# linjieli222/HERO

Hardware: AMD Instinct MI355X
Metric: videos/sec training step, HERO-base TVR-shaped batch (higher is better)
Workload: dtype bf16; 1 GPU; configs[1]: HERO-base TVR finetune micro-step (train-tvr-8gpu.json shapes: 32 videos x 60 frames, 15 subs x (4 frames + 20 tokens), 15-token query; vfeat 4352; fwd + VSM loss + bwd, all-reduce/clip/AdamW every 2nd micro-step); global_batch=32, parallelism=dp1, grad_accum=2, launch=hipGraph replay, input=one batch resident in HBM

## Files before the change

hero_amd/_lib.py:

```python
import ctypes as C
import os

import torch

_HERE = os.path.dirname(os.path.abspath(__file__))
LIB_PATH = os.environ.get("HERO_HIP_LIB") or os.path.join(_HERE, "libhero_hip.so")

ABI_VERSION = 3
F32, BF16 = 0, 1
LAYOUT_K, LAYOUT_O = 0, 1
ACT_NONE, ACT_GELU, ACT_RELU, ACT_GELU_BWD, ACT_RELU_BWD, ACT_GELU_DG, ACT_MUL_AUX = 0, 1, 2, 3, 4, 5, 6

EXPORTS = [
    "hero_last_error", "hero_abi_version", "hero_abi_struct_count", "hero_abi_struct_bytes", "hero_gemm", "hero_gemm_splits", "hero_fold_slabs", "hero_wgrad_group", "hero_wgrad_batch_plan", "hero_wgrad_batch", "hero_prof_enable", "hero_prof_read", "hero_probe_mfma", "hero_probe_hbm", "hero_gemm_force_config", "hero_layernorm_fwd",
    "hero_layernorm_bwd_workspace_bytes", "hero_layernorm_bwd", "hero_colsum_workspace_bytes",
    "hero_colsum", "hero_colsum_multi", "hero_colsum_multi_workspace_bytes", "hero_layernorm_bwd_blocks", "hero_attention_fwd", "hero_attention_bwd", "hero_attention_max_len", "hero_attention_max_packed_len", "hero_attention_stats_ok", "hero_attention_force_ppw",
    "hero_gather_rows", "hero_inverse_first", "hero_csr_gather_sum", "hero_scatter_add_rows", "hero_segment_sort_workspace_bytes", "hero_scatter_add_sorted_workspace_bytes", "hero_segment_sort", "hero_scatter_add_sorted", "hero_cast", "hero_transpose_cast", "hero_copy_multi",
    "hero_relu_bwd", "hero_gelu_bwd", "hero_add", "hero_sumsq", "hero_adamw", "hero_adamw_multi", "hero_adamw_multi_chunk",
    "hero_query_pool_fwd", "hero_query_pool_bwd", "hero_rownorm_fwd", "hero_rownorm_bwd", "hero_score_max_fwd",
    "hero_score_max_bwd", "hero_rank_loss", "hero_sums_scaled", "hero_st_ed_fwd", "hero_st_ed_bwd", "hero_st_ed_bwd_workspace_bytes",
    "hero_cross_entropy_fwd", "hero_cross_entropy_bwd", "hero_qa_pool_fwd", "hero_qa_pool_bwd",
    "hero_topk_rows", "hero_st_ed_probs", "hero_moment_topk", "hero_moment_nms", "hero_first_hit",
    "hero_collate_subs", "hero_collate_clip_mask", "hero_collate_frame_map", "hero_collate_gather_feats", "hero_derive_multi",
    "hero_comm_available", "hero_comm_unique_id", "hero_comm_init", "hero_comm_destroy", "hero_comm_rank", "hero_comm_world",
    "hero_comm_allreduce_buckets", "hero_comm_broadcast", "hero_comm_allgather", "hero_comm_allgather_var",
]


class Dropout(C.Structure):
    _fields_ = [("seed_ptr", C.c_void_p), ("site", C.c_uint64),
                ("threshold16", C.c_uint32), ("scale", C.c_float)]


class GemmEpilogue(C.Structure):
    _fields_ = [("bias", C.c_void_p), ("residual", C.c_void_p), ("aux", C.c_void_p),
                ("act", C.c_int), ("out_f32", C.c_int), ("beta", C.c_float),
                ("split_k", C.c_int), ("dropout", Dropout), ("colsum", C.c_void_p), ("colsum_partial", C.c_int), ("pad_", C.c_int), ("split_stride", C.c_longlong)]


class CrossEntropy(C.Structure):
    _fields_ = [("logits", C.c_void_p), ("labels", C.c_void_p), ("loss", C.c_void_p), ("lse", C.c_void_p),
                ("dloss", C.c_void_p), ("dlogits", C.c_void_p), ("rows", C.c_int), ("cols", C.c_int),
                ("ld", C.c_int), ("dtype", C.c_int), ("inv_temp", C.c_float), ("ignore_index", C.c_int64)]


class Derive(C.Structure):
    _fields_ = [("src", C.c_void_p), ("dst", C.c_void_p), ("n", C.c_int64), ("mode", C.c_int), ("p0", C.c_int),
                ("p1", C.c_int), ("p2", C.c_int)]


DERIVE_MASK_ADD, DERIVE_F32, DERIVE_I32, DERIVE_FLAT_GATHER = 0, 1, 2, 3


class WgradProblem(C.Structure):
    _fields_ = [("dy", C.c_void_p), ("x", C.c_void_p), ("dw", C.c_void_p), ("M", C.c_int), ("N", C.c_int),
                ("ld_dy", C.c_int), ("ld_x", C.c_int), ("ld_dw", C.c_int), ("split_hint", C.c_int), ("dbias", C.c_void_p)]


class LnFwd(C.Structure):
    _fields_ = [("x", C.c_void_p), ("tab", C.c_void_p * 3), ("idx", C.c_void_p * 3),
                ("gamma", C.c_void_p), ("beta", C.c_void_p), ("y", C.c_void_p),
                ("pre", C.c_void_p), ("mean", C.c_void_p), ("rstd", C.c_void_p),
                ("rows", C.c_int), ("cols", C.c_int), ("eps", C.c_float),
                ("x_dtype", C.c_int), ("y_dtype", C.c_int), ("dropout", Dropout)]


class LnBwd(C.Structure):
    _fields_ = [("x", C.c_void_p), ("dy", C.c_void_p), ("gamma", C.c_void_p),
                ("mean", C.c_void_p), ("rstd", C.c_void_p), ("dx", C.c_void_p),
                ("dx_dropped", C.c_void_p), ("dgamma", C.c_void_p), ("dbeta", C.c_void_p),
                ("grad_beta", C.c_float), ("workspace", C.c_void_p),
                ("rows", C.c_int), ("cols", C.c_int), ("x_dtype", C.c_int), ("dtype", C.c_int),
                ("dropout_out", Dropout), ("dropout_in", Dropout), ("dbias_in", C.c_void_p), ("defer_fold", C.c_int)]


class Colsum(C.Structure):
    _fields_ = [("src", C.c_void_p), ("dst", C.c_void_p), ("rows", C.c_int), ("cols", C.c_int), ("ld", C.c_int),
                ("dtype", C.c_int), ("beta", C.c_float), ("row_cols", C.c_int), ("dst_rows", C.c_void_p)]


class Attn(C.Structure):
    _fields_ = [("qkv", C.c_void_p), ("mask", C.c_void_p), ("ctx", C.c_void_p),
                ("probs", C.c_void_p), ("dctx", C.c_void_p), ("dqkv", C.c_void_p),
                ("S", C.c_int), ("L", C.c_int), ("H", C.c_int), ("scale", C.c_float),
                ("dtype", C.c_int), ("dropout", Dropout), ("seq_off", C.c_void_p), ("stats", C.c_void_p)]


class AdamW(C.Structure):
    _fields_ = [("p", C.c_void_p), ("g", C.c_void_p), ("m", C.c_void_p), ("v", C.c_void_p),
                ("n", C.c_size_t), ("lr", C.c_float), ("beta1", C.c_float), ("beta2", C.c_float),
                ("eps", C.c_float), ("weight_decay", C.c_float), ("step", C.c_int),
                ("grad_sumsq", C.c_void_p), ("max_grad_norm", C.c_float),
                ("grad_scale", C.c_float), ("shadow", C.c_void_p)]


class TensorDesc(C.Structure):
    _fields_ = [("p", C.c_void_p), ("g", C.c_void_p), ("m", C.c_void_p), ("v", C.c_void_p),
                ("n", C.c_uint64), ("group", C.c_int32), ("step_lag", C.c_int32)]


class AdamWGroup(C.Structure):
    _fields_ = [("lr", C.c_float), ("beta1", C.c_float), ("beta2", C.c_float), ("eps", C.c_float),
                ("weight_decay", C.c_float)]


class AdamWMulti(C.Structure):
    _fields_ = [("descs", C.c_void_p), ("chunk_tensor", C.c_void_p), ("chunk_index", C.c_void_p),
                ("n_chunks", C.c_int), ("groups", AdamWGroup * 8), ("step", C.c_int),
                ("grad_sumsq", C.c_void_p), ("max_grad_norm", C.c_float), ("grad_scale", C.c_float),
                ("step_ptr", C.c_void_p), ("lr_ptr", C.c_void_p), ("tensor_steps", C.c_void_p), ("n_tensors", C.c_int)]


class CopyDesc(C.Structure):
    _fields_ = [("src", C.c_void_p), ("dst", C.c_void_p), ("rows", C.c_int32), ("cols", C.c_int32),
                ("ldd", C.c_int32), ("transpose", C.c_int32), ("dst_dtype", C.c_int32), ("pad_", C.c_int32)]


class QueryPool(C.Structure):
    _fields_ = [("q", C.c_void_p), ("mask", C.c_void_p), ("w", C.c_void_p), ("pooled", C.c_void_p),
                ("att", C.c_void_p), ("dpooled", C.c_void_p), ("dq", C.c_void_p), ("dw", C.c_void_p),
                ("B", C.c_int), ("L", C.c_int), ("D", C.c_int), ("dtype", C.c_int)]


class RowNorm(C.Structure):
    _fields_ = [("x", C.c_void_p), ("y", C.c_void_p), ("rnorm", C.c_void_p), ("dy", C.c_void_p),
                ("dx", C.c_void_p), ("rows", C.c_int), ("cols", C.c_int), ("x_dtype", C.c_int),
                ("eps", C.c_float)]


class ScoreMax(C.Structure):
    _fields_ = [("s", C.c_void_p), ("mask", C.c_void_p), ("out", C.c_void_p), ("arg", C.c_void_p),
                ("ds_ctx", C.c_void_p), ("ds_q", C.c_void_p), ("gc", C.c_void_p), ("gq", C.c_void_p),
                ("qn", C.c_void_p), ("cn", C.c_void_p), ("dqn", C.c_void_p), ("dcn", C.c_void_p),
                ("M", C.c_int), ("N", C.c_int), ("L", C.c_int), ("D", C.c_int), ("n0", C.c_int),
                ("n_own", C.c_int), ("ld_s", C.c_int), ("gc_scale", C.c_float), ("gq_scale", C.c_float)]


class RankLoss(C.Structure):
    _fields_ = [("s", C.c_void_p), ("loss_ctx_rows", C.c_void_p), ("loss_q_rows", C.c_void_p),
                ("ds_ctx", C.c_void_p), ("ds_q", C.c_void_p), ("nq", C.c_int), ("nv", C.c_int),
                ("margin", C.c_float), ("lse", C.c_int), ("hard", C.c_int), ("pool", C.c_int),
                ("hard_w", C.c_float), ("easy_w", C.c_float)]


class StEd(C.Structure):
    _fields_ = [("q2", C.c_void_p), ("ctx", C.c_void_p), ("mask", C.c_void_p), ("w_st", C.c_void_p),
                ("w_ed", C.c_void_p), ("targets", C.c_void_p), ("loss_rows", C.c_void_p),
                ("p_st", C.c_void_p), ("p_ed", C.c_void_p), ("sim", C.c_void_p), ("g", C.c_void_p),
                ("dq2", C.c_void_p), ("dctx", C.c_void_p), ("dw_st", C.c_void_p), ("dw_ed", C.c_void_p),
                ("B", C.c_int), ("L", C.c_int), ("D", C.c_int), ("K", C.c_int), ("dtype", C.c_int), ("g_scale", C.c_float),
                ("ws", C.c_void_p)]


class CommBucket(C.Structure):
    _fields_ = [("buf", C.c_void_p), ("count", C.c_size_t), ("dtype", C.c_int), ("pad_", C.c_int)]


ABI_STRUCTS = [Dropout, GemmEpilogue, WgradProblem, LnFwd, LnBwd, Colsum, Attn, AdamW, TensorDesc, AdamWGroup, AdamWMulti,
               CopyDesc, QueryPool, RowNorm, ScoreMax, RankLoss, StEd, CrossEntropy, Derive, CommBucket]


def abi_struct_sizes():
    return {st.__name__: C.sizeof(st) for st in ABI_STRUCTS}


_lib = None


def lib():
    global _lib
    if _lib is None:
        if not os.path.exists(LIB_PATH):
            raise RuntimeError(
                "hero_amd: %s is missing. Build it with `python -m hero_amd.build` "
                "(needs hipcc; cross-compiles for gfx950 without a GPU). There is no fallback "
                "path." % LIB_PATH)
        L = C.CDLL(LIB_PATH)
        L.hero_last_error.restype = C.c_char_p
        have = L.hero_abi_version()
        if have != ABI_VERSION:
            raise RuntimeError("hero_amd: %s reports ABI version %d, this binding was written against %d (struct layouts "
                               "differ: rebuild with `python -m hero_amd.build --force`)" % (LIB_PATH, have, ABI_VERSION))
        L.hero_abi_struct_bytes.argtypes = [C.c_int]
        if L.hero_abi_struct_count() != len(ABI_STRUCTS):
            raise RuntimeError("hero_amd: %s declares %d ABI structs, this binding mirrors %d" % (LIB_PATH, L.hero_abi_struct_count(), len(ABI_STRUCTS)))
        bad = [(st.__name__, C.sizeof(st), L.hero_abi_struct_bytes(i)) for i, st in enumerate(ABI_STRUCTS)
               if C.sizeof(st) != L.hero_abi_struct_bytes(i)]
        if bad:
            raise RuntimeError("hero_amd: struct layouts differ from %s (name, binding bytes, library bytes): %s" % (LIB_PATH, bad))
        L.hero_layernorm_bwd_workspace_bytes.restype = C.c_size_t
        L.hero_colsum_workspace_bytes.restype = C.c_size_t
        L.hero_colsum_multi_workspace_bytes.restype = C.c_size_t
        L.hero_colsum_multi_workspace_bytes.argtypes = [C.POINTER(Colsum), C.c_int]
        L.hero_colsum_multi.argtypes = [C.POINTER(Colsum), C.c_int, C.c_void_p, C.c_void_p]
        L.hero_layernorm_bwd_blocks.argtypes = [C.c_int]
        L.hero_gemm.argtypes = [C.c_void_p, C.c_void_p, C.c_void_p] + [C.c_int] * 9 + [
            C.POINTER(GemmEpilogue), C.c_void_p]
        L.hero_gemm_splits.argtypes = [C.c_int, C.c_int, C.c_int]
        L.hero_fold_slabs.argtypes = [C.c_void_p, C.c_int, C.c_size_t, C.c_void_p, C.c_size_t, C.c_int, C.c_void_p]
        L.hero_wgrad_group.argtypes = [C.POINTER(WgradProblem), C.c_int, C.c_int, C.c_int, C.c_void_p]
        L.hero_wgrad_batch_plan.argtypes = [C.POINTER(WgradProblem), C.c_int, C.c_int, C.c_void_p, C.c_int]
        L.hero_wgrad_batch.argtypes = [C.POINTER(WgradProblem), C.c_int, C.c_int, C.c_int, C.c_void_p, C.c_int, C.c_void_p]
        L.hero_prof_enable.argtypes = [C.c_int]
        L.hero_prof_read.argtypes = [C.c_int, C.POINTER(C.c_double), C.POINTER(C.c_double),
                                     C.POINTER(C.c_longlong)]
        L.hero_probe_mfma.argtypes = [C.c_void_p, C.c_size_t, C.POINTER(C.c_double), C.POINTER(C.c_double), C.c_void_p]
        L.hero_probe_hbm.argtypes = [C.c_void_p, C.c_void_p, C.c_size_t, C.POINTER(C.c_double), C.POINTER(C.c_double), C.c_void_p]
        L.hero_layernorm_fwd.argtypes = [C.POINTER(LnFwd), C.c_void_p]
        L.hero_layernorm_bwd.argtypes = [C.POINTER(LnBwd), C.c_void_p]
        L.hero_layernorm_bwd_workspace_bytes.argtypes = [C.c_int, C.c_int]
        L.hero_colsum_workspace_bytes.argtypes = [C.c_int, C.c_int]
        L.hero_colsum.argtypes = [C.c_void_p, C.c_void_p, C.c_int, C.c_int, C.c_int, C.c_int,
                                  C.c_float, C.c_void_p, C.c_void_p]
        L.hero_attention_fwd.argtypes = [C.POINTER(Attn), C.c_void_p]
        L.hero_attention_bwd.argtypes = [C.POINTER(Attn), C.c_void_p]
        L.hero_attention_stats_ok.argtypes = [C.c_int, C.c_int]
        L.hero_attention_force_ppw.argtypes = [C.c_int]
        L.hero_attention_max_len.argtypes = [C.c_int, C.c_int]
        L.hero_attention_max_packed_len.argtypes = [C.c_int]
        L.hero_gather_rows.argtypes = [C.c_void_p, C.c_void_p, C.c_void_p, C.c_void_p,
                                       C.c_int, C.c_int, C.c_int, C.c_void_p]
        L.hero_inverse_first.argtypes = [C.c_void_p, C.c_int, C.c_void_p, C.c_int, C.c_int, C.c_void_p]
        L.hero_csr_gather_sum.argtypes = [C.c_void_p, C.c_void_p, C.c_void_p, C.c_void_p,
                                          C.c_int, C.c_int, C.c_int, C.c_void_p]
        L.hero_scatter_add_rows.argtypes = [C.c_void_p, C.c_void_p, C.c_void_p, C.c_void_p,
                                            C.c_int, C.c_int, C.c_int, C.c_int, C.c_int, C.c_void_p]
        L.hero_segment_sort_workspace_bytes.argtypes = [C.c_int]
        L.hero_segment_sort_workspace_bytes.restype = C.c_size_t
        L.hero_segment_sort.argtypes = [C.c_void_p, C.c_int, C.c_int, C.c_int, C.c_void_p, C.c_void_p, C.c_void_p]
        L.hero_scatter_add_sorted_workspace_bytes.argtypes = [C.c_int, C.c_int]
        L.hero_scatter_add_sorted_workspace_bytes.restype = C.c_size_t
        L.hero_scatter_add_sorted.argtypes = [C.c_void_p, C.c_void_p, C.c_void_p, C.c_void_p, C.c_int, C.c_int, C.c_int, C.c_int,
                                              C.c_void_p, C.c_void_p]
        L.hero_st_ed_bwd_workspace_bytes.argtypes = [C.c_int]
        L.hero_st_ed_bwd_workspace_bytes.restype = C.c_size_t
        L.hero_cast.argtypes = [C.c_void_p, C.c_void_p, C.c_size_t, C.c_int, C.c_int, C.c_void_p]
        L.hero_transpose_cast.argtypes = [C.c_void_p, C.c_void_p, C.c_int, C.c_int, C.c_int, C.c_int,
                                          C.c_void_p]
        L.hero_relu_bwd.argtypes = [C.c_void_p, C.c_void_p, C.c_void_p, C.c_size_t, C.c_int,
                                    C.c_void_p]
        L.hero_gelu_bwd.argtypes = L.hero_relu_bwd.argtypes
        L.hero_add.argtypes = [C.c_void_p, C.c_void_p, C.c_void_p, C.c_size_t, C.c_int, C.c_void_p]
        L.hero_sumsq.argtypes = [C.c_void_p, C.c_size_t, C.c_void_p, C.c_void_p, C.c_void_p]
        L.hero_adamw.argtypes = [C.POINTER(AdamW), C.c_void_p]
        L.hero_adamw_multi.argtypes = [C.POINTER(AdamWMulti), C.c_void_p]
        L.hero_copy_multi.argtypes = [C.c_void_p, C.c_void_p, C.c_void_p, C.c_int, C.c_void_p]
        for fn, st in (("hero_query_pool_fwd", QueryPool), ("hero_query_pool_bwd", QueryPool),
                       ("hero_rownorm_fwd", RowNorm), ("hero_rownorm_bwd", RowNorm),
                       ("hero_score_max_fwd", ScoreMax), ("hero_score_max_bwd", ScoreMax),
                       ("hero_rank_loss", RankLoss), ("hero_st_ed_fwd", StEd), ("hero_st_ed_bwd", StEd)):
            getattr(L, fn).argtypes = [C.POINTER(st), C.c_void_p]
        L.hero_sums_scaled.argtypes = [C.c_void_p, C.c_int, C.c_int, C.POINTER(C.c_float), C.c_void_p, C.c_void_p]
        L.hero_topk_rows.argtypes = [C.c_void_p, C.c_int, C.c_int, C.c_int, C.c_int, C.c_float, C.c_void_p, C.c_void_p, C.c_void_p]
        L.hero_st_ed_probs.argtypes = [C.c_void_p, C.c_longlong] + [C.c_void_p] * 4 + [C.c_int] * 5 + [C.c_void_p] * 3
        L.hero_moment_topk.argtypes = [C.c_void_p] * 3 + [C.c_int] * 6 + [C.c_void_p] * 3
        L.hero_moment_nms.argtypes = [C.c_void_p] * 3 + [C.c_int, C.c_int, C.c_double, C.c_int, C.c_int] + [C.c_void_p] * 3
        L.hero_first_hit.argtypes = [C.c_void_p] * 3 + [C.c_int] * 3 + [C.c_void_p, C.c_void_p, C.c_float, C.c_void_p, C.c_int, C.c_void_p, C.c_void_p]
        L.hero_collate_subs.argtypes = [C.c_void_p] * 4 + [C.c_int] * 3 + [C.c_void_p]
        L.hero_collate_gather_feats.argtypes = [C.c_void_p] * 7 + [C.c_int] * 5 + [C.c_void_p]
        L.hero_derive_multi.argtypes = [C.POINTER(Derive), C.c_int, C.c_void_p]
        L.hero_collate_clip_mask.argtypes = [C.c_void_p, C.c_void_p, C.c_int, C.c_int, C.c_void_p]
        L.hero_collate_frame_map.argtypes = [C.c_void_p] * 7 + [C.c_int] * 4 + [C.c_void_p]
        L.hero_cross_entropy_fwd.argtypes = [C.POINTER(CrossEntropy), C.c_void_p]
        L.hero_cross_entropy_bwd.argtypes = [C.POINTER(CrossEntropy), C.c_void_p]
        L.hero_qa_pool_fwd.argtypes = [C.c_void_p] * 8 + [C.c_int] * 6 + [C.c_void_p]
        L.hero_qa_pool_bwd.argtypes = [C.c_void_p] * 11 + [C.c_int] * 6 + [C.c_void_p]
        L.hero_comm_unique_id.argtypes = [C.c_void_p]
        L.hero_comm_init.argtypes = [C.c_void_p, C.c_int, C.c_int, C.POINTER(C.c_void_p)]
        L.hero_comm_destroy.argtypes = [C.c_void_p]
        L.hero_comm_rank.argtypes = [C.c_void_p]
        L.hero_comm_world.argtypes = [C.c_void_p]
        L.hero_comm_allreduce_buckets.argtypes = [C.c_void_p, C.POINTER(CommBucket), C.c_int, C.c_void_p]
        L.hero_comm_broadcast.argtypes = [C.c_void_p, C.c_void_p, C.c_size_t, C.c_int, C.c_void_p]
        L.hero_comm_allgather.argtypes = [C.c_void_p, C.c_void_p, C.c_void_p, C.c_size_t, C.c_void_p]
        L.hero_comm_allgather_var.argtypes = [C.c_void_p, C.c_void_p, C.c_void_p, C.POINTER(C.c_size_t), C.c_void_p]
        _lib = L
    return _lib


def check(rc):
    if rc != 0:
        raise RuntimeError("libhero_hip: %s (code %d)" % (lib().hero_last_error().decode(), rc))


def dt(t):
    if t.dtype == torch.float32:
        return F32
    if t.dtype == torch.bfloat16:
        return BF16
    raise TypeError("hero_amd: unsupported dtype %s (float32 / bfloat16 only)" % t.dtype)


def ptr(t):
    if t is None:
        return None
    if not t.is_cuda:
        raise RuntimeError("hero_amd: tensor is on %s; the HIP path needs CUDA/ROCm tensors and has "
                           "no CPU fallback" % t.device)
    if not t.is_contiguous():
        raise RuntimeError("hero_amd: non-contiguous tensor passed to a HIP kernel")
    return t.data_ptr()


_raw_stream = getattr(torch._C, "_cuda_getCurrentRawStream", None)
_cur_device = getattr(torch._C, "_cuda_getDevice", None)


def stream():
    if _raw_stream is not None and _cur_device is not None:
        return _raw_stream(_cur_device())
    return torch.cuda.current_stream().cuda_stream


def no_dropout():
    return Dropout(None, 0, 0, 1.0)
```

hero_amd/build.py:

```python
import os
import shutil
import subprocess
import sys
from concurrent.futures import ThreadPoolExecutor

HERE = os.path.dirname(os.path.abspath(__file__))
CSRC = os.path.join(HERE, "csrc")
OBJ = os.path.join(CSRC, "_obj")
LIB = os.path.join(HERE, "libhero_hip.so")
SOURCES = ["api.cpp", "comm.cpp", "gemm.hip", "gemm_ws.hip", "layernorm.hip", "attention.hip", "attention_mfma.hip", "attention_mfma_long.hip", "rows.hip", "head.hip", "qa_pool.hip", "retrieval.hip", "postproc.hip", "loss.hip", "collate.hip", "probe.hip"]
FLAGS = ["--offload-arch=gfx950", "-O3", "-std=c++17", "-fPIC", "-Wall", "-Wno-unused-function",
         "-ffp-contract=off"]


def _hipcc():
    exe = shutil.which("hipcc") or "/opt/rocm/bin/hipcc"
    if not os.path.exists(exe):
        raise RuntimeError("hipcc not found: cannot build libhero_hip.so")
    return exe


def _stale(target, deps):
    if not os.path.exists(target):
        return True
    t = os.path.getmtime(target)
    return any(os.path.getmtime(d) > t for d in deps)


def build(force=False, verbose=False):
    os.makedirs(OBJ, exist_ok=True)
    hipcc = _hipcc()
    headers = [os.path.join(CSRC, "common.h"), os.path.join(CSRC, "gemm_args.h"), os.path.join(CSRC, "gemm_ws_common.h"), os.path.join(CSRC, "attn_mfma.h"),
               os.path.join(os.path.dirname(HERE), "include", "hero_hip.h")]
    jobs = []
    objs = []
    for src in SOURCES:
        s = os.path.join(CSRC, src)
        o = os.path.join(OBJ, os.path.splitext(src)[0] + ".o")
        objs.append(o)
        if force or _stale(o, [s] + headers):
            jobs.append([hipcc, "-x", "hip"] + FLAGS + ["-c", s, "-o", o])

    def run(cmd):
        if verbose:
            print(" ".join(cmd), flush=True)
        r = subprocess.run(cmd, capture_output=True, text=True)
        if r.returncode != 0:
            raise RuntimeError("hipcc failed:\n%s\n%s" % (" ".join(cmd), r.stderr[-4000:]))
        if verbose and r.stderr.strip():
            print(r.stderr, file=sys.stderr)

    for f in os.listdir(OBJ):
        if f.endswith(".o") and os.path.join(OBJ, f) not in objs:
            os.remove(os.path.join(OBJ, f))
    with ThreadPoolExecutor(max_workers=4) as ex:
        list(ex.map(run, jobs))
    if jobs or force or _stale(LIB, objs):
        run([hipcc, "--offload-arch=gfx950", "-shared", "-fPIC", "-o", LIB] + objs + ["-ldl"])
    return LIB


if __name__ == "__main__":
    print(build(force="--force" in sys.argv, verbose=True))
```

hero_amd/csrc/gemm.hip:

```cpp
#include "gemm_args.h"
#include <vector>

namespace hero {

typedef __attribute__((ext_vector_type(8))) short bf16x8_t;
typedef __attribute__((ext_vector_type(16))) float f32x16_t;

__device__ __forceinline__ int swz(int row) { return (row ^ (row >> 3)) & 7; }

template <typename T> struct Tr;
template <> struct Tr<bf16_t> { static constexpr int BK = 64, EPC = 8; };
template <> struct Tr<float>  { static constexpr int BK = 32, EPC = 4; };

template <int WM_, int WN_, int TM_, int TN_> struct Cfg {
  static constexpr int WM = WM_, WN = WN_, TM = TM_, TN = TN_;
  static constexpr int NT = 64 * WM * WN;
  static constexpr int BM = WM * TM * 32, BN = WN * TN * 32;
  static constexpr int A_BYTES = BM * 128, B_BYTES = BN * 128, STAGE = A_BYTES + B_BYTES;
  static constexpr int EPI_ROWS = BM < 128 ? BM : (BM % 128 == 0 ? 128 : BM / 2);
  static constexpr int EPI_BYTES = EPI_ROWS * BN * 4;
  static constexpr int LDS = 2 * STAGE > EPI_BYTES ? 2 * STAGE : EPI_BYTES;
};

template <typename T, int LAY, int R, int NT> struct Stage;
// ... 757 lines not shown
  return check_launch("hero_gemm");
}

static int pick_cfg(int M, int N, int split, bool k_contig) {
  if (g_force_cfg >= 0 && g_force_cfg < 8) return g_force_cfg;
  if (!k_contig || split != 1) return 0;
  const long long t128 = (long long)((M + 127) / 128) * ((N + 127) / 128);
  if (t128 <= 192) return 3;
  if (t128 > 512 && t128 <= 700 && (long long)((M + 191) / 192) * ((N + 127) / 128) <= 512) return 1;
  const long long tiles = (long long)((M + 255) / 256) * ((N + 255) / 256);
  const long long rounds = (tiles + 255) / 256;
  return (tiles >= 256 && tiles * 10 >= rounds * 256 * 9) ? 2 : 0;
}

static int g_use_glds = 1;

#define HERO_GLDS_INST(T, CF)                                                       \
  template __global__ void gemm_glds_kernel<T, CF, EK_GENERIC>(GemmArgs);           \
  template __global__ void gemm_glds_kernel<T, CF, 0>(GemmArgs);                    \
  template __global__ void gemm_glds_kernel<T, CF, EK_BIAS>(GemmArgs);              \
  template __global__ void gemm_glds_kernel<T, CF, EK_BIAS | EK_RES | EK_DROP>(GemmArgs); \
  template __global__ void gemm_glds_kernel<T, CF, EK_BIAS | EK_GELU>(GemmArgs);    \
  template __global__ void gemm_glds_kernel<T, CF, EK_RES>(GemmArgs);               \
  template __global__ void gemm_glds_kernel<T, CF, EK_GELU_BWD>(GemmArgs);
HERO_GLDS_INST(bf16_t, Cfg128)
HERO_GLDS_INST(bf16_t, Cfg256)
HERO_GLDS_INST(bf16_t, Cfg64)
HERO_GLDS_INST(bf16_t, Cfg192)
template __global__ void gemm_glds_kernel<float, Cfg192, EK_GENERIC>(GemmArgs);
template __global__ void gemm_glds_kernel<float, Cfg64, EK_GENERIC>(GemmArgs);
template __global__ void gemm_glds_kernel<float, Cfg128, EK_GENERIC>(GemmArgs);
template __global__ void gemm_glds_kernel<float, Cfg256, EK_GENERIC>(GemmArgs);

template <typename T, typename CF, int EK>
static int launch_glds_ek(GemmArgs g, hipStream_t s) {
  HERO_ENSURE_LDS((&gemm_glds_kernel<T, CF, EK>), GldsRing<CF>::LDS, "gemm_glds_kernel");
  g.tiles_m = (g.M + CF::BM - 1) / CF::BM;
  g.tiles_n = (g.N + CF::BN - 1) / CF::BN;
  const int split = g.epi.split_k > 1 ? g.epi.split_k : 1;
  const int grid = g.tiles_m * g.tiles_n * split;
  ProfSlot* ps = nullptr;
  hipEvent_t e0 = nullptr, e1 = nullptr;
  if (g_prof_on) {
    ps = &g_prof[(sizeof(T) == 2 ? 4 : 0)];
    if (ps->flops.size() < 16384 && hipEventCreate(&e0) == hipSuccess && hipEventCreate(&e1) == hipSuccess) {
      (void)hipEventRecord(e0, s);
    } else {
      ps = nullptr;
    }
  }
  hipLaunchKernelGGL((gemm_glds_kernel<T, CF, EK>), dim3(grid), dim3(CF::NT), GldsRing<CF>::LDS, s, g);
  if (ps) {
    (void)hipEventRecord(e1, s);
    ps->ev.push_back(e0);
    ps->ev.push_back(e1);
    ps->flops.push_back(2.0 * (double)g.M * (double)g.N * (double)g.K);
  }
  return check_launch("hero_gemm(glds)");
}

template <typename T, typename CF>
static int launch_glds(const GemmArgs& g, hipStream_t s) {
  const HeroGemmEpilogue& e = g.epi;
  if constexpr (sizeof(T) == 2) if (!e.out_f32 && e.split_k <= 1) {
    const bool b = e.bias != nullptr, r = e.residual != nullptr, d = e.dropout.threshold16 != 0;
    if (e.act == HERO_ACT_NONE && b && !r && !d) return launch_glds_ek<T, CF, EK_BIAS>(g, s);
    if (e.act == HERO_ACT_NONE && b && r) return launch_glds_ek<T, CF, EK_BIAS | EK_RES | EK_DROP>(g, s);
    if ((e.act == HERO_ACT_GELU || e.act == HERO_ACT_GELU_DG) && b && !r && !d) return launch_glds_ek<T, CF, EK_BIAS | EK_GELU>(g, s);
    if (e.act == HERO_ACT_NONE && !b && !r && !d) return launch_glds_ek<T, CF, 0>(g, s);
    if (e.act == HERO_ACT_NONE && !b && r && !d) return launch_glds_ek<T, CF, EK_RES>(g, s);
    if ((e.act == HERO_ACT_GELU_BWD || e.act == HERO_ACT_MUL_AUX) && !b && !r && !d) return launch_glds_ek<T, CF, EK_GELU_BWD>(g, s);
  }
  return launch_glds_ek<T, CF, EK_GENERIC>(g, s);
}

static int launch_glds_tr(GemmArgs g, hipStream_t s) {
  typedef Cfg<2, 2, 2, 2> CF;
  g.tiles_m = (g.M + CF::BM - 1) / CF::BM;
  g.tiles_n = (g.N + CF::BN - 1) / CF::BN;
  const int split = g.epi.split_k > 1 ? g.epi.split_k : 1;
  const int grid = g.tiles_m * g.tiles_n * split;
  ProfSlot* ps = nullptr;
  hipEvent_t e0 = nullptr, e1 = nullptr;
  if (g_prof_on) {
    ps = &g_prof[7];
    if (ps->flops.size() < 16384 && hipEventCreate(&e0) == hipSuccess && hipEventCreate(&e1) == hipSuccess) {
      (void)hipEventRecord(e0, s);
    } else {
      ps = nullptr;
    }
  }
  HERO_ENSURE_LDS(&gemm_glds_tr_kernel, 65536, "gemm_glds_tr_kernel");
  hipLaunchKernelGGL(gemm_glds_tr_kernel, dim3(grid), dim3(256), 65536, s, g);
  if (ps) {
    (void)hipEventRecord(e1, s);
    ps->ev.push_back(e0);
    ps->ev.push_back(e1);
    ps->flops.push_back(2.0 * (double)g.M * (double)g.N * (double)g.K);
  }
  return check_launch("hero_gemm(glds_tr)");
}

template <typename T, int AL, int BL>
static int launch_cfg(const GemmArgs& g, int cfg, hipStream_t s) {
  if (AL == HERO_LAYOUT_O && BL == HERO_LAYOUT_O && sizeof(T) == 2 && g_use_glds && g.K > 0 && g.k_per_split % 64 == 0)
    return launch_glds_tr(g, s);
  if (AL == HERO_LAYOUT_K && BL == HERO_LAYOUT_K && g_use_glds && g.K > 0 && g.K % Tr<T>::BK == 0 &&
      g.k_per_split % Tr<T>::BK == 0) {
    if (cfg == 2) return launch_glds<T, Cfg256>(g, s);
    if (cfg == 3) return launch_glds<T, Cfg64>(g, s);
    if (cfg == 1) return launch_glds<T, Cfg192>(g, s);
    return launch_glds<T, Cfg128>(g, s);
  }
  if (cfg == 2) return launch<T, AL, BL, Cfg256>(g, s);
  return launch<T, AL, BL, Cfg128>(g, s);
}

template <typename T>
static int dispatch(const GemmArgs& g, int al, int bl, int cfg, hipStream_t s) {
  if (al == HERO_LAYOUT_K && bl == HERO_LAYOUT_K) return launch_cfg<T, HERO_LAYOUT_K, HERO_LAYOUT_K>(g, cfg, s);
  if (al == HERO_LAYOUT_K && bl == HERO_LAYOUT_O) return launch_cfg<T, HERO_LAYOUT_K, HERO_LAYOUT_O>(g, cfg, s);
  if (al == HERO_LAYOUT_O && bl == HERO_LAYOUT_O) return launch_cfg<T, HERO_LAYOUT_O, HERO_LAYOUT_O>(g, cfg, s);
  if (al == HERO_LAYOUT_O && bl == HERO_LAYOUT_K) return launch_cfg<T, HERO_LAYOUT_O, HERO_LAYOUT_K>(g, cfg, s);
  set_error("hero_gemm: bad layout (%d, %d)", al, bl);
  return HERO_ERR_ARG;
}

}

using namespace hero;

template <int CTRL, int ROW_MASK>
__device__ __forceinline__ float dpp_add(float v) {
  return v + __builtin_bit_cast(float, __builtin_amdgcn_update_dpp(0, __builtin_bit_cast(int, v), CTRL, ROW_MASK, 0xf, false));
}
__device__ __forceinline__ float wave_sum_lane63(float v) {
  v = dpp_add<0xb1, 0xf>(v);
  v = dpp_add<0x4e, 0xf>(v);
  v = dpp_add<0x124, 0xf>(v);
  v = dpp_add<0x128, 0xf>(v);
  v = dpp_add<0x142, 0xa>(v);
  v = dpp_add<0x143, 0xc>(v);
  return v;
}

__global__ __launch_bounds__(256) void gemm_skinny_f32_kernel(const float* __restrict__ A, const float* __restrict__ B, float* __restrict__ C,
                                                              const float* __restrict__ bias, int M, int N, int K, int lda, int ldb, int ldc) {
  extern __shared__ __attribute__((aligned(16))) char smem_skinny[];
  float* xs = reinterpret_cast<float*>(smem_skinny);
  constexpr int KC = 1024;
  const int lane = threadIdx.x & 63, wave = threadIdx.x >> 6;
  const int n0 = (blockIdx.x * 4 + wave) * 2;
  const bool live = n0 < N, two = n0 + 1 < N;
  float acc0[32], acc1[32];
#pragma unroll
  for (int m = 0; m < 32; ++m) acc0[m] = acc1[m] = 0.f;
  const float* b0 = B + (size_t)(live ? n0 : 0) * ldb;
  const float* b1 = B + (size_t)(two ? n0 + 1 : (live ? n0 : 0)) * ldb;
  for (int kc = 0; kc < K; kc += KC) {
    const int kw = min(KC, K - kc);
    float4 w0[4], w1[4];
#pragma unroll
    for (int j = 0; j < 4; ++j) {
      const int k = min(lane * 4 + j * 256, kw - 4);
      w0[j] = *reinterpret_cast<const float4*>(b0 + kc + k);
      w1[j] = *reinterpret_cast<const float4*>(b1 + kc + k);
    }
    if (kc) __syncthreads();
    {
      const int k = threadIdx.x * 4;
      const bool in = k < kw;
      const float* src = A + kc + (in ? k : 0);
      float* dst = in ? xs + k : xs + 32 * kw;
      const int dstride = in ? kw : 0;
#pragma unroll
      for (int m0 = 0; m0 < 32; m0 += 16) {
        float4 t[16];
#pragma unroll
        for (int j = 0; j < 16; ++j) t[j] = *reinterpret_cast<const float4*>(src + (size_t)(m0 + j < M ? m0 + j : M - 1) * lda);
#pragma unroll
        for (int j = 0; j < 16; ++j) *reinterpret_cast<float4*>(dst + (m0 + j) * dstride) = t[j];
      }
    }
    __syncthreads();
    if (live) {
#pragma unroll
      for (int j = 0; j < 4; ++j) {
        const int k = lane * 4 + j * 256;
        if (k < kw) {
#pragma unroll
          for (int m0 = 0; m0 < 32; m0 += 16) {
            float4 xv[16];
#pragma unroll
            for (int q = 0; q < 16; ++q) xv[q] = *reinterpret_cast<const float4*>(xs + (m0 + q) * kw + k);
            __builtin_amdgcn_sched_barrier(0);
#pragma unroll
            for (int q = 0; q < 16; ++q) {
              const float4 x = xv[q];
              acc0[m0 + q] = fmaf(x.w, w0[j].w, fmaf(x.z, w0[j].z, fmaf(x.y, w0[j].y, fmaf(x.x, w0[j].x, acc0[m0 + q]))));
              acc1[m0 + q] = fmaf(x.w, w1[j].w, fmaf(x.z, w1[j].z, fmaf(x.y, w1[j].y, fmaf(x.x, w1[j].x, acc1[m0 + q]))));
            }
            __builtin_amdgcn_sched_barrier(0);
          }
        }
      }
    }
  }
  if (!live) return;
  float v0 = 0.f, v1 = 0.f;
#pragma unroll
  for (int m = 0; m < 32; ++m) {
    const float s0 = __builtin_bit_cast(float, __builtin_amdgcn_readlane(__builtin_bit_cast(int, wave_sum_lane63(acc0[m])), 63));
    const float s1 = __builtin_bit_cast(float, __builtin_amdgcn_readlane(__builtin_bit_cast(int, wave_sum_lane63(acc1[m])), 63));
    v0 = lane == m ? s0 : v0;
    v1 = lane == m ? s1 : v1;
  }
  if (lane < M) {
    C[(size_t)lane * ldc + n0] = v0 + (bias ? bias[n0] : 0.f);
    if (two) C[(size_t)lane * ldc + n0 + 1] = v1 + (bias ? bias[n0 + 1] : 0.f);
  }
}

extern "C" int hero_gemm(const void* A, const void* B, void* C, int M, int N, int K, int lda, int ldb, int ldc,
                         int a_layout, int b_layout, int dtype, const HeroGemmEpilogue* epi, hero_stream_t stream) {
  HERO_REQUIRE(A && B && C && epi, "hero_gemm: null pointer");
  HERO_REQUIRE(dtype == HERO_F32 || dtype == HERO_BF16, "hero_gemm: bad dtype %d", dtype);
  if (M <= 0 || N <= 0) return HERO_OK;
  HERO_REQUIRE(K >= 0, "hero_gemm: K < 0");
  const int vec = dtype == HERO_BF16 ? 8 : 4;
  HERO_REQUIRE(N % 4 == 0 && ldc % 4 == 0, "hero_gemm: N (%d) and ldc (%d) must be multiples of 4", N, ldc);
  HERO_REQUIRE(lda % vec == 0 && ldb % vec == 0, "hero_gemm: lda/ldb (%d, %d) must be multiples of %d", lda, ldb, vec);
  HERO_REQUIRE(a_layout == HERO_LAYOUT_K ? K % vec == 0 : M % vec == 0,
               "hero_gemm: A contiguous dim must be a multiple of %d (M=%d K=%d layout=%d)", vec, M, K, a_layout);
  HERO_REQUIRE(b_layout == HERO_LAYOUT_K ? K % vec == 0 : N % vec == 0,
               "hero_gemm: B contiguous dim must be a multiple of %d (N=%d K=%d layout=%d)", vec, N, K, b_layout);
  HERO_REQUIRE((((uintptr_t)A | (uintptr_t)B | (uintptr_t)C) & 15) == 0, "hero_gemm: operands must be 16-byte aligned");
  HERO_REQUIRE(!epi->residual || (((uintptr_t)epi->residual) & 7) == 0, "hero_gemm: residual misaligned");
  HERO_REQUIRE(!(epi->act == HERO_ACT_GELU || epi->act == HERO_ACT_GELU_BWD || epi->act == HERO_ACT_RELU_BWD || epi->act == HERO_ACT_GELU_DG ||
                 epi->act == HERO_ACT_MUL_AUX) || epi->aux,
               "hero_gemm: activation %d needs aux", epi->act);
  HERO_REQUIRE(!epi->colsum || (epi->split_k <= 1 && !epi->out_f32), "hero_gemm: epilogue.colsum excludes split_k / out_f32");
  HERO_REQUIRE(epi->split_stride == 0 || (epi->split_k > 1 && epi->split_stride >= (long long)(M - 1) * ldc + N),
               "hero_gemm: split_stride needs split_k > 1 and slabs that hold [M, ldc]");
  GemmArgs g;
  g.A = A; g.B = B; g.C = C;
  g.M = M; g.N = N; g.K = K; g.lda = lda; g.ldb = ldb; g.ldc = ldc;
  g.tiles_m = g.tiles_n = 0;
  g.group = g_group ? g_group : (N >= 2560 ? 16 : (N <= 1024 ? 4 : 8));
  g.epi = *epi;
  const int bk = dtype == HERO_BF16 ? 64 : 32;
  const bool k_contig = a_layout == HERO_LAYOUT_K && b_layout == HERO_LAYOUT_K;
  hipStream_t s = static_cast<hipStream_t>(stream);
  if (dtype == HERO_F32 && k_contig && M <= 32 && K >= 256 && g_force_cfg == -1 && epi->act == HERO_ACT_NONE && !epi->residual && !epi->colsum &&
      !epi->out_f32 && epi->split_k <= 1 && epi->dropout.threshold16 == 0) {
    void* tok = gemm_prof_begin(3, s);
    const int lds = 32 * (K < 1024 ? K : 1024) * 4 + 16;
    HERO_ENSURE_LDS(&gemm_skinny_f32_kernel, 32 * 1024 * 4 + 16, "gemm_skinny_f32_kernel");
    hipLaunchKernelGGL(gemm_skinny_f32_kernel, dim3((N + 7) / 8), dim3(256), lds, s, static_cast<const float*>(A), static_cast<const float*>(B),
                       static_cast<float*>(C), epi->bias, M, N, K, lda, ldb, ldc);
    gemm_prof_end(tok, 2.0 * (double)M * (double)N * (double)K, s);
    return check_launch("hero_gemm(skinny f32)");
  }
  if (dtype == HERO_BF16) {
    const int rc = gemm_ws_run(A, B, C, M, N, K, lda, ldb, ldc, a_layout, b_layout, *epi, g_force_cfg, s);
    if (rc != -1) return rc;
  }
  if (epi->split_k > 1) {
    HERO_REQUIRE(epi->out_f32 && epi->act == HERO_ACT_NONE && !epi->bias && !epi->residual && epi->dropout.threshold16 == 0,
                 "hero_gemm: split_k supports only a plain fp32 accumulate epilogue");
    const int ktiles = (K + bk - 1) / bk;
    int split = epi->split_k < ktiles ? epi->split_k : ktiles;
    if (split > 1) {
      const int per = (ktiles + split - 1) / split;
      split = (ktiles + per - 1) / per;
      if (split > 1) {
        if (epi->split_stride == 0 && epi->beta != 1.f) {
          hipLaunchKernelGGL(scale_f32_kernel, dim3(1024), dim3(256), 0, s, static_cast<float*>(C), M, N, ldc, epi->beta);
          const int rc = check_launch("hero_gemm(scale)");
          if (rc) return rc;
        }
        g.k_per_split = per * bk;
        g.epi.split_k = split;
        const int cfg = pick_cfg(M, N, split, k_contig);
        return dtype == HERO_BF16 ? dispatch<bf16_t>(g, a_layout, b_layout, cfg, s) : dispatch<float>(g, a_layout, b_layout, cfg, s);
      }
    }
  }
  g.k_per_split = K > 0 ? ((K + bk - 1) / bk) * bk : bk;
  g.epi.split_k = 1;
  const int cfg = pick_cfg(M, N, 1, k_contig);
  return dtype == HERO_BF16 ? dispatch<bf16_t>(g, a_layout, b_layout, cfg, s) : dispatch<float>(g, a_layout, b_layout, cfg, s);
}

extern "C" int hero_gemm_splits(int K, int split_k, int dtype) {
  const int bk = dtype == HERO_BF16 ? 64 : 32;
  const int ktiles = (K + bk - 1) / bk;
  int split = split_k < ktiles ? split_k : ktiles;
  if (split <= 1) return 1;
  const int per = (ktiles + split - 1) / split;
  return (ktiles + per - 1) / per;
}

extern "C" int hero_gemm_force_config(int cfg) {
  if (cfg >= 8 && cfg <= 14 && cfg != 11 && cfg != 12) {
    g_force_cfg = cfg;
    g_use_glds = 1;
    g_group = 0;
    return HERO_OK;
  }
  g_force_cfg = cfg >= 0 ? (cfg & 3) : -1;
  g_use_glds = cfg >= 0 ? !(cfg & 4) : 1;
  g_group = cfg >= 0 ? (cfg >> 8) : 0;
  return HERO_OK;
}

extern "C" int hero_prof_enable(int on) {
  for (auto& p : g_prof) {
    for (hipEvent_t e : p.ev) (void)hipEventDestroy(e);
    p.ev.clear();
    p.flops.clear();
  }
  g_prof_on = on != 0;
  return HERO_OK;
}
extern "C" int hero_prof_read(int slot, double* total_ms, double* total_flops, long long* launches) {
  HERO_REQUIRE(slot >= 0 && slot < 11 && total_ms && total_flops && launches, "hero_prof_read: bad arguments");
  ProfSlot& p = g_prof[slot];
  double ms = 0.0, fl = 0.0;
  for (size_t i = 0; i < p.flops.size(); ++i) {
    float t = 0.f;
    if (hipEventSynchronize(p.ev[2 * i + 1]) != hipSuccess || hipEventElapsedTime(&t, p.ev[2 * i], p.ev[2 * i + 1]) != hipSuccess) {
      set_error("hero_prof_read: event query failed");
      return HERO_ERR_LAUNCH;
    }
    ms += t;
    fl += p.flops[i];
  }
  *total_ms = ms;
  *total_flops = fl;
  *launches = (long long)p.flops.size();
  return HERO_OK;
}
```

hero_amd/csrc/gemm_ws.hip:

```cpp
#include <stdlib.h>
#include <type_traits>

#include "gemm_ws_common.h"

namespace hero {
namespace ws {

template <int TM, int TN, bool TR, int EK>
__global__ __launch_bounds__(512) __attribute__((amdgpu_waves_per_eu(2, 2))) void gemm_ws_kernel(WsArgs g) {
  typedef Geo<TM, TN> G;
  extern __shared__ __attribute__((aligned(16))) char smem[];
  const int lane = threadIdx.x & 63;
  const int wave = __builtin_amdgcn_readfirstlane(threadIdx.x >> 6);
  const int nwg = gridDim.x;
  int wg;
  {
    const int bid = blockIdx.x, q = nwg >> 3, r = nwg & 7, xcd = bid & 7, loc = bid >> 3;
    wg = (xcd < r ? xcd * (q + 1) : r * (q + 1) + (xcd - r) * q) + loc;
  }

  if (wave >= 4) {
    Loader<G, TR> ld(g, smem, wg, nwg, wave - 4, lane);
    constexpr int AHEAD = (G::NSG - 2) * G::PW;
    bool more = ld.issue();
#pragma unroll
    for (int k = 0; k < G::NSG - 2; ++k) more = ld.issue();
    if (more) wait_vm<AHEAD>(); else wait_vm<0>();
    __builtin_amdgcn_s_barrier();
    unsigned slot = 0;
    int item_no = 0;
    for (int cit = wg; cit < g.nwork; cit += nwg, ++item_no) {
      const Item ic = item_coord<G>(g, cit);
      WS_T(item_no, 0, wave, lane);
      for (int t = 0; t < ic.nk; ++t) {
        if (ld.issue()) wait_vm<AHEAD>(); else wait_vm<0>();
        __builtin_amdgcn_s_barrier();
        if (t + 1 < ic.nk) { slot += G::STAGE; if (slot == G::NSG * G::STAGE) slot = 0; }
      }
      WS_T(item_no, 1, wave, lane);
#ifndef HERO_WS_NOEPI
      if constexpr (!TR) epilogue_rows<G, EK, false>(g, ic, smem, slot, nullptr, wave, lane, item_no);
#endif
      slot += G::STAGE; if (slot == G::NSG * G::STAGE) slot = 0;
    }
    return;
  }

  const int wm = wave >> 1, wn = wave & 1;
  const int arow0 = wm * TM * 32, brow0 = wn * TN * 32;
  unsigned ao[TM], bo[TN];
  if (!TR) {
    const int r = lane & 31, kg = lane >> 5;
#pragma unroll
    for (int i = 0; i < TM; ++i) { const int ra = arow0 + i * 32 + r; ao[i] = ra * 128 + ((kg ^ swz_k(ra)) << 4); }
#pragma unroll
    for (int j = 0; j < TN; ++j) { const int rb = brow0 + j * 32 + r; bo[j] = G::A_BYTES + rb * 128 + ((kg ^ swz_k(rb)) << 4); }
  } else {
    const int p = lane & 15, gq = (lane >> 4) & 1, kg = lane >> 5;
    const int krow = kg * 8 + (p >> 2);
#pragma unroll
    for (int i = 0; i < TM; ++i) {
      const int col = arow0 + i * 32 + gq * 16 + 4 * (p & 3);
      ao[i] = krow * (G::BM * 2) + ((((col >> 3) ^ swz_o<G::BM * 2>(krow)) << 4) | ((col & 7) * 2));
    }
#pragma unroll
    for (int j = 0; j < TN; ++j) {
      const int col = brow0 + j * 32 + gq * 16 + 4 * (p & 3);
      bo[j] = G::A_BYTES + krow * (G::BN * 2) + ((((col >> 3) ^ swz_o<G::BN * 2>(krow)) << 4) | ((col & 7) * 2));
    }
  }
  bf16x8_t a0[TM], b0[TN], a1[TM], b1[TN];
  auto ldf = [&](bf16x8_t (&a)[TM], bf16x8_t (&b)[TN], const char* st, int ks) {
    typedef __attribute__((address_space(3))) bf16x4_t* lp_t;
    auto ra = [&](int i) {
      if (!TR) {
        a[i] = *reinterpret_cast<const bf16x8_t*>(st + (ao[i] ^ (ks << 5)));
      } else {
        const char* q = st + ao[i] + ks * 16 * (G::BM * 2);
        const bf16x4_t lo = __builtin_amdgcn_ds_read_tr16_b64_v4i16((lp_t)(q));
        const bf16x4_t hi = __builtin_amdgcn_ds_read_tr16_b64_v4i16((lp_t)(q + 4 * (G::BM * 2)));
        a[i] = bf16x8_t{lo[0], lo[1], lo[2], lo[3], hi[0], hi[1], hi[2], hi[3]};
      }
    };
    auto rb = [&](int j) {
      if (!TR) {
        b[j] = *reinterpret_cast<const bf16x8_t*>(st + (bo[j] ^ (ks << 5)));
      } else {
        const char* q = st + bo[j] + ks * 16 * (G::BN * 2);
        const bf16x4_t lo = __builtin_amdgcn_ds_read_tr16_b64_v4i16((lp_t)(q));
        const bf16x4_t hi = __builtin_amdgcn_ds_read_tr16_b64_v4i16((lp_t)(q + 4 * (G::BN * 2)));
        b[j] = bf16x8_t{lo[0], lo[1], lo[2], lo[3], hi[0], hi[1], hi[2], hi[3]};
      }
    };
    if (!TR) {
      ra(0);
#pragma unroll
      for (int j = 0; j < TN; ++j) rb(j);
#pragma unroll
      for (int i = 1; i < TM; ++i) ra(i);
    } else {
      ra(0);
#pragma unroll
      for (int j = 0; j < TN; ++j) rb(j);
#pragma unroll
      for (int i = 1; i < TM; ++i) ra(i);
    }
  };
  f32x16_t acc[TM][TN];
  auto mma = [&](const bf16x8_t (&a)[TM], const bf16x8_t (&b)[TN]) {
#pragma unroll
    for (int i = 0; i < TM; ++i)
#pragma unroll
      for (int j = 0; j < TN; ++j) {
        if (!TR) acc[i][j] = __builtin_amdgcn_mfma_f32_32x32x16_bf16(b[j], a[i], acc[i][j], 0, 0, 0);
        else acc[i][j] = __builtin_amdgcn_mfma_f32_32x32x16_bf16(a[i], b[j], acc[i][j], 0, 0, 0);
      }
  };

  __builtin_amdgcn_s_setprio(2);
  __builtin_amdgcn_s_barrier();
  unsigned curo = 0;
  if (wg < g.nwork) ldf(a0, b0, smem, 0);
  int item_no = 0;
  for (int cit = wg; cit < g.nwork; cit += nwg, ++item_no) {
    const Item ic = item_coord<G>(g, cit);
    WS_T(item_no, 0, wave, lane);
#pragma unroll
    for (int i = 0; i < TM; ++i)
#pragma unroll
      for (int j = 0; j < TN; ++j)
#pragma unroll
        for (int e = 0; e < 16; ++e) acc[i][j][e] = 0.f;
    const bool more_items = cit + nwg < g.nwork;
    unsigned last = curo;
    for (int t = 0; t < ic.nk; ++t) {
      const char* cur = smem + curo;
      last = curo;
      curo += G::STAGE;
      if (curo == G::NSG * G::STAGE) curo = 0;
      const char* nxt = smem + curo;
      constexpr int NRD = TR ? 2 * (TM + TN) : TM + TN;
      ldf(a1, b1, cur, 1);
      mma(a0, b0);
      WS_INTERLEAVE(TM * TN, NRD);
      __builtin_amdgcn_sched_barrier(0);
      ldf(a0, b0, cur, 2);
      mma(a1, b1);
      WS_INTERLEAVE(TM * TN, NRD);
      __builtin_amdgcn_sched_barrier(0);
      ldf(a1, b1, cur, 3);
      mma(a0, b0);
      WS_INTERLEAVE(TM * TN, NRD);
      __builtin_amdgcn_sched_barrier(0);
      wait_lds();
      __builtin_amdgcn_s_barrier();
      __builtin_amdgcn_sched_barrier(0);
      ldf(a0, b0, nxt, 0);
      mma(a1, b1);
      WS_INTERLEAVE(TM * TN, NRD);
      __builtin_amdgcn_sched_barrier(0);
    }
    if constexpr (!TR) {
      __builtin_amdgcn_s_setprio(0);
      WS_T(item_no, 1, wave, lane);
#ifndef HERO_WS_NOEPI
      epilogue_rows<G, EK, true>(g, ic, smem, last, acc, wave, lane, item_no);
#else
      {
        float sum = 0.f;
#pragma unroll
        for (int i = 0; i < TM; ++i)
#pragma unroll
          for (int j = 0; j < TN; ++j)
#pragma unroll
            for (int e = 0; e < 16; ++e) sum += acc[i][j][e];
        if (sum == 1.2345e-30f) static_cast<bf16_t*>(g.C)[lane] = (bf16_t)1;
      }
#endif
      __builtin_amdgcn_s_setprio(2);
      if (more_items) ldf(a0, b0, smem + curo, 0);
    } else {
      float* C = static_cast<float*>(g.C);
#pragma unroll
      for (int i = 0; i < TM; ++i)
#pragma unroll
        for (int j = 0; j < TN; ++j) {
          const int gn = ic.n0 + brow0 + j * 32 + (lane & 31);
#pragma unroll
          for (int r = 0; r < 16; ++r) {
            const int gm = ic.m0 + arow0 + i * 32 + (r & 3) + 8 * (r >> 2) + 4 * (lane >> 5);
            if (gm < g.M && gn < g.N) atomicAdd(C + (size_t)gm * g.ldc + gn, acc[i][j][r]);
          }
        }
    }
  }
}

struct WsgProb {
  const bf16_t* A;
  const bf16_t* B;
  float* C;
  int M, N, lda, ldb, ldc, tiles_n, tile0;
};
struct WsgArgs {
  WsgProb p[4];
  int nprob, K, ksteps, total_tiles;
};
struct Seg { int prob, m0, n0, k0, nk; };

template <typename G>
__device__ __forceinline__ Seg seg_at(const WsgArgs& g, int pos, int end) {
  const int tile = pos / g.ksteps, k0 = pos - tile * g.ksteps;
  int pi = 0;
#pragma unroll
  for (int q = 1; q < 4; ++q)
    if (q < g.nprob && tile >= g.p[q].tile0) pi = q;
  const int t = tile - g.p[pi].tile0;
  Seg s;
  s.prob = pi;
  s.m0 = (t / g.p[pi].tiles_n) * G::BM;
  s.n0 = (t % g.p[pi].tiles_n) * G::BN;
  s.k0 = k0;
  s.nk = min(g.ksteps - k0, end - pos);
  return s;
}

__global__ __launch_bounds__(512) __attribute__((amdgpu_waves_per_eu(2, 2))) void gemm_wsg_kernel(WsgArgs g) {
  typedef Geo<3, 3> G;
  constexpr int TM = 3, TN = 3;
  extern __shared__ __attribute__((aligned(16))) char smem[];
  const int lane = threadIdx.x & 63;
  const int wave = __builtin_amdgcn_readfirstlane(threadIdx.x >> 6);
  const int nwg = gridDim.x;
  int wg;
  {
    const int bid = blockIdx.x, q = nwg >> 3, r = nwg & 7, xcd = bid & 7, loc = bid >> 3;
    wg = (xcd < r ? xcd * (q + 1) : r * (q + 1) + (xcd - r) * q) + loc;
  }
  const long long total = (long long)g.total_tiles * g.ksteps;
  const int start = (int)(total * wg / nwg), end = (int)(total * (wg + 1) / nwg);
  if (start >= end) return;

  if (wave >= 4) {
    const int w = wave - 4;
    constexpr int CA = G::BM / 8, CB = G::BN / 8;
    int pos = start;
    Seg sg = seg_at<G>(g, pos, end);
    int ik = 0;
    unsigned goa[G::PA], gob[G::PB];
    const char* pa = nullptr;
    const char* pb = nullptr;
    unsigned ra_left = 0, rb_left = 0, sa = 0, sb = 0, fill = 0;
    auto setup = [&]() {
      const WsgProb& P = g.p[sg.prob];
#pragma unroll
      for (int i = 0; i < G::PA; ++i) {
        const int id = (w * G::PA + i) * 64 + lane, row = id / CA, c = (id % CA) ^ swz_o<G::BM * 2>(row);
        goa[i] = (unsigned)row * (unsigned)P.lda * 2u + (c << 4);
      }
#pragma unroll
      for (int i = 0; i < G::PB; ++i) {
        const int id = (w * G::PB + i) * 64 + lane, row = id / CB, c = (id % CB) ^ swz_o<G::BN * 2>(row);
        gob[i] = (unsigned)row * (unsigned)P.ldb * 2u + (c << 4);
      }
      const int kb = sg.k0 * 64;
      pa = reinterpret_cast<const char*>(P.A + (size_t)kb * P.lda + sg.m0);
      pb = reinterpret_cast<const char*>(P.B + (size_t)kb * P.ldb + sg.n0);
      ra_left = (unsigned)(((size_t)(g.K - kb) * P.lda - sg.m0) * 2);
      rb_left = (unsigned)(((size_t)(g.K - kb) * P.ldb - sg.n0) * 2);
      sa = 64u * (unsigned)P.lda * 2u;
      sb = 64u * (unsigned)P.ldb * 2u;
    };
    setup();
    auto issue = [&]() -> bool {
      if (pos >= end) return false;
      char* buf = smem + fill;
      const __amdgpu_buffer_rsrc_t ra = __builtin_amdgcn_make_buffer_rsrc(const_cast<char*>(pa), 0, ra_left, 0x00020000);
      const __amdgpu_buffer_rsrc_t rb = __builtin_amdgcn_make_buffer_rsrc(const_cast<char*>(pb), 0, rb_left, 0x00020000);
#pragma unroll
      for (int i = 0; i < G::PA; ++i)
        __builtin_amdgcn_raw_ptr_buffer_load_lds(ra, HERO_LDS_PTR(buf + (w * G::PA + i) * 1024), 16, goa[i], 0, 0, HERO_WS_LOAD_AUX_A);
#pragma unroll
      for (int i = 0; i < G::PB; ++i)
        __builtin_amdgcn_raw_ptr_buffer_load_lds(rb, HERO_LDS_PTR(buf + G::A_BYTES + (w * G::PB + i) * 1024), 16, gob[i], 0, 0, HERO_WS_LOAD_AUX_B);
      fill += G::STAGE;
      if (fill == NS * G::STAGE) fill = 0;
      ++pos;
      if (++ik == sg.nk) {
        ik = 0;
        if (pos < end) { sg = seg_at<G>(g, pos, end); setup(); }
      } else {
        pa += sa; pb += sb;
        ra_left = ra_left > sa ? ra_left - sa : 0u;
        rb_left = rb_left > sb ? rb_left - sb : 0u;
      }
      return true;
    };
    issue();
    const bool second = issue();
    if (second) wait_vm<G::PW>(); else wait_vm<0>();
    __builtin_amdgcn_s_barrier();
    for (int u = start; u < end; ++u) {
      if (issue()) wait_vm<G::PW>(); else wait_vm<0>();
      __builtin_amdgcn_s_barrier();
    }
    return;
  }

  const int wm = wave >> 1, wn = wave & 1;
  const int arow0 = wm * TM * 32, brow0 = wn * TN * 32;
  unsigned ao[TM], bo[TN];
  {
    const int p = lane & 15, gq = (lane >> 4) & 1, kg = lane >> 5;
    const int krow = kg * 8 + (p >> 2);
#pragma unroll
    for (int i = 0; i < TM; ++i) {
      const int col = arow0 + i * 32 + gq * 16 + 4 * (p & 3);
      ao[i] = krow * (G::BM * 2) + ((((col >> 3) ^ swz_o<G::BM * 2>(krow)) << 4) | ((col & 7) * 2));
    }
#pragma unroll
    for (int j = 0; j < TN; ++j) {
      const int col = brow0 + j * 32 + gq * 16 + 4 * (p & 3);
      bo[j] = G::A_BYTES + krow * (G::BN * 2) + ((((col >> 3) ^ swz_o<G::BN * 2>(krow)) << 4) | ((col & 7) * 2));
    }
  }
  typedef __attribute__((address_space(3))) bf16x4_t* lp_t;
  bf16x8_t a0[TM], b0[TN], a1[TM], b1[TN];
  auto ldf = [&](bf16x8_t (&a)[TM], bf16x8_t (&b)[TN], const char* st, int ks) {
    auto ra = [&](int i) {
      const char* q = st + ao[i] + ks * 16 * (G::BM * 2);
      const bf16x4_t lo = __builtin_amdgcn_ds_read_tr16_b64_v4i16((lp_t)(q));
      const bf16x4_t hi = __builtin_amdgcn_ds_read_tr16_b64_v4i16((lp_t)(q + 4 * (G::BM * 2)));
      a[i] = bf16x8_t{lo[0], lo[1], lo[2], lo[3], hi[0], hi[1], hi[2], hi[3]};
    };
    ra(0);
#pragma unroll
    for (int j = 0; j < TN; ++j) {
      const char* q = st + bo[j] + ks * 16 * (G::BN * 2);
      const bf16x4_t lo = __builtin_amdgcn_ds_read_tr16_b64_v4i16((lp_t)(q));
      const bf16x4_t hi = __builtin_amdgcn_ds_read_tr16_b64_v4i16((lp_t)(q + 4 * (G::BN * 2)));
      b[j] = bf16x8_t{lo[0], lo[1], lo[2], lo[3], hi[0], hi[1], hi[2], hi[3]};
    }
#pragma unroll
    for (int i = 1; i < TM; ++i) ra(i);
  };
  f32x16_t acc[TM][TN];
  auto mma = [&](const bf16x8_t (&a)[TM], const bf16x8_t (&b)[TN]) {
#pragma unroll
    for (int i = 0; i < TM; ++i)
#pragma unroll
      for (int j = 0; j < TN; ++j) acc[i][j] = __builtin_amdgcn_mfma_f32_32x32x16_bf16(a[i], b[j], acc[i][j], 0, 0, 0);
  };
  __builtin_amdgcn_s_setprio(2);
  __builtin_amdgcn_s_barrier();
  unsigned curo = 0;
  ldf(a0, b0, smem, 0);
  [[maybe_unused]] int seg_no = 0;
  for (int pos = start; pos < end; ++seg_no) {
    const Seg sg = seg_at<G>(g, pos, end);
    WS_T(seg_no, 0, wave, lane);
#pragma unroll
    for (int i = 0; i < TM; ++i)
#pragma unroll
      for (int j = 0; j < TN; ++j)
#pragma unroll
        for (int e = 0; e < 16; ++e) acc[i][j][e] = 0.f;
    for (int t = 0; t < sg.nk; ++t) {
      const char* cur = smem + curo;
      curo += G::STAGE;
      if (curo == NS * G::STAGE) curo = 0;
      const char* nxt = smem + curo;
      ldf(a1, b1, cur, 1);
      mma(a0, b0);
      WS_INTERLEAVE(TM * TN, 2 * (TM + TN));
      __builtin_amdgcn_sched_barrier(0);
      ldf(a0, b0, cur, 2);
      mma(a1, b1);
      WS_INTERLEAVE(TM * TN, 2 * (TM + TN));
      __builtin_amdgcn_sched_barrier(0);
      ldf(a1, b1, cur, 3);
      mma(a0, b0);
      WS_INTERLEAVE(TM * TN, 2 * (TM + TN));
      __builtin_amdgcn_sched_barrier(0);
      wait_lds();
      __builtin_amdgcn_s_barrier();
      __builtin_amdgcn_sched_barrier(0);
      ldf(a0, b0, nxt, 0);
      mma(a1, b1);
      WS_INTERLEAVE(TM * TN, 2 * (TM + TN));
      __builtin_amdgcn_sched_barrier(0);
    }
    pos += sg.nk;
    WS_T(seg_no, 1, wave, lane);
#ifdef HERO_WS_TRACE
    if (blockIdx.x == 0 && lane == 0 && seg_no < 4) g_ws_trace[(seg_no * 16 + 3) * 8 + wave] = (unsigned long long)sg.nk;
#endif
    const WsgProb& P = g.p[sg.prob];
#pragma unroll
    for (int i = 0; i < TM; ++i)
#pragma unroll
      for (int j = 0; j < TN; ++j) {
        const int gn = sg.n0 + brow0 + j * 32 + (lane & 31);
#pragma unroll
        for (int r = 0; r < 16; ++r) {
          const int gm = sg.m0 + arow0 + i * 32 + (r & 3) + 8 * (r >> 2) + 4 * (lane >> 5);
          if (gm < P.M && gn < P.N) atomicAdd(P.C + (size_t)gm * P.ldc + gn, acc[i][j][r]);
        }
      }
    WS_T(seg_no, 14, wave, lane);
  }
}

struct WsbProb {
  const bf16_t* A;
  const bf16_t* B;
  float* C;
  float* colsum;
  int M, N, lda, ldb, ldc, pad_;
};
struct WsbItem { int prob, m0, n0, k0, nk, order, nslices, flag; };
struct WsbArgs {
  const WsbItem* items;
  int* flags;
  int rounds, K, nprob, pad_;
  WsbProb p[HERO_WGRAD_BATCH_MAX];
};

template <typename G, bool COMPUTE>
__device__ __forceinline__ void epilogue_acc(const WsbProb& P, const WsbItem& it, int* flags, char* smem, unsigned slot,
                                             f32x16_t (*acc)[G::TN], int wave, int lane, bool want_cs = false) {
  constexpr int TM = G::TM, TN = G::TN, BN = G::BN, RPP = G::RPP, C8 = G::C8, RPI = G::RPI, ITERS = G::ITERS;
  char* st = smem + slot;
  int tid = threadIdx.x;
  asm volatile("" : "+v"(tid));
  lane = tid & 63;
  wave = __builtin_amdgcn_readfirstlane(tid >> 6);
  const int c8 = tid % C8, r0 = tid / C8;
  const int gn = it.n0 + c8 * 8;
  const bool col_ok = r0 < RPI && gn < P.N;
  const int wm = wave >> 1, wn = wave & 1, l31 = lane & 31, half = lane >> 5;
  const bool plain = it.nslices == 1;
  constexpr bool SPLIT = (RPP == 64 && G::PASSES == TM);
  auto tile_row = [](int p, int row) { return SPLIT ? (row >> 5) * (TM * 32) + p * 32 + (row & 31) : p * RPP + row; };
  const __amdgpu_buffer_rsrc_t rc = __builtin_amdgcn_make_buffer_rsrc(P.C, 0, 0x7ffffff0, 0x00020000);
  if (!plain && it.order > 0) {
    if (lane == 0)
      while (__hip_atomic_load(flags + it.flag, __ATOMIC_RELAXED, __HIP_MEMORY_SCOPE_AGENT) != it.order) __builtin_amdgcn_s_sleep(8);
  }
#pragma unroll
  for (int p = 0; p < G::PASSES; ++p) {
    u32x4_t old0[ITERS], old1[ITERS];
    unsigned voff[ITERS];
    if (plain) {
#pragma unroll
      for (int i = 0; i < ITERS; ++i) {
        const int row = r0 + i * RPI;
        const int gm = it.m0 + tile_row(p, row);
        const bool ok = col_ok && row < RPP && gm < P.M;
        voff[i] = ok ? ((unsigned)gm * (unsigned)P.ldc + (unsigned)gn) * 4u : 0xfffffff0u;
#if defined(HERO_WSB_EPI_NOLOAD) || defined(HERO_WSB_EPI_NOMEM)
        old0[i] = u32x4_t{0u, 0u, 0u, 0u};
        old1[i] = u32x4_t{0u, 0u, 0u, 0u};
#else
        old0[i] = __builtin_amdgcn_raw_buffer_load_b128(rc, voff[i], 0, 0);
        old1[i] = __builtin_amdgcn_raw_buffer_load_b128(rc, voff[i], 16, 0);
#endif
      }
    }
    if constexpr (COMPUTE) {
#pragma unroll
      for (int b = 0; b < RPP / 32; ++b) {
        const int blk = SPLIT ? b * TM + p : p * (RPP / 32) + b;
        if (wm == blk / TM) {
          const int i = blk % TM;
#pragma unroll
          for (int j = 0; j < TN; ++j)
#pragma unroll
            for (int q = 0; q < 4; ++q) {
              const int chunk = (wn * TN * 32 + j * 32 + 8 * q + 4 * half) >> 2;
              const f32x4_t v = {acc[i][j][4 * q], acc[i][j][4 * q + 1], acc[i][j][4 * q + 2], acc[i][j][4 * q + 3]};
              *reinterpret_cast<f32x4_t*>(st + (32 * b + l31) * G::ROWB + ((chunk ^ (l31 & 7)) << 4)) = v;
            }
        }
      }
    }
    wait_lds();
    __builtin_amdgcn_s_barrier();
    if constexpr (!COMPUTE) {
      if (p == 0 && want_cs && tid - 256 < G::BM) {
        const int c = tid - 256, gm = it.m0 + c;
        const float* sp = reinterpret_cast<const float*>(smem + SPARE_OFF);
        const float sum = sp[c];
        if (gm < P.M) {
          if (plain) P.colsum[gm] += sum; else atomicAdd(P.colsum + gm, sum);
        }
      }
    }
    if (plain) {
// ... 15 lines not shown
          }
#ifdef HERO_WSB_EPI_NOMEM
        asm volatile("" ::"v"(v0[0]), "v"(v1[0]), "v"(v0[1]), "v"(v1[1]));
        continue;
#endif
#pragma unroll
        for (int i = 0; i < 2; ++i) {
          __builtin_amdgcn_raw_buffer_store_b128(u32x4_t{__float_as_uint(v0[i][0]), __float_as_uint(v0[i][1]), __float_as_uint(v0[i][2]), __float_as_uint(v0[i][3])}, rc, voff[h + i], 0, HERO_WS_STORE_DW);
          __builtin_amdgcn_raw_buffer_store_b128(u32x4_t{__float_as_uint(v1[i][0]), __float_as_uint(v1[i][1]), __float_as_uint(v1[i][2]), __float_as_uint(v1[i][3])}, rc, voff[h + i], 16, HERO_WS_STORE_DW);
        }
      }
    } else {
      const int col = tid % BN, rr = tid / BN;
      const int gc = it.n0 + col;
      if (tid < 2 * BN && gc < P.N) {
        const unsigned sw = (unsigned)(col >> 2);
#pragma unroll 4
        for (int q = 0; q < RPP / 2; ++q) {
          const int row = 2 * q + rr;
          const int gm = it.m0 + tile_row(p, row);
          const float v = *reinterpret_cast<const float*>(st + row * G::ROWB + (((sw ^ (unsigned)(row & 7))) << 4) + (col & 3) * 4);
          if (gm < P.M) atomicAdd(P.C + (size_t)gm * P.ldc + gc, v);
        }
      }
      if (p == G::PASSES - 1) wait_vm<0>();
    }
    wait_lds();
    __builtin_amdgcn_s_barrier();
  }
  if (!plain && tid == 0)
    __hip_atomic_store(flags + it.flag, it.order + 1 < it.nslices ? it.order + 1 : 0, __ATOMIC_RELAXED, __HIP_MEMORY_SCOPE_AGENT);
}

__global__ __launch_bounds__(512) __attribute__((amdgpu_waves_per_eu(2, 2))) void gemm_wsb_kernel(WsbArgs g) {
  typedef Geo<3, 3> G;
  constexpr int TM = 3, TN = 3;
  extern __shared__ __attribute__((aligned(16))) char smem[];
  const int lane = threadIdx.x & 63;
  const int wave = __builtin_amdgcn_readfirstlane(threadIdx.x >> 6);
  const int nwg = gridDim.x;
  int wg;
  {
    const int bid = blockIdx.x, q = nwg >> 3, r = nwg & 7, xcd = bid & 7, loc = bid >> 3;
    wg = (xcd < r ? xcd * (q + 1) : r * (q + 1) + (xcd - r) * q) + loc;
  }
  auto next_round = [&](int r) {
    while (r < g.rounds && g.items[(size_t)r * nwg + wg].nk == 0) ++r;
    return r;
  };

  if (wave >= 4) {
    const int w = wave - 4;
    constexpr int CA = G::BM / 8, CB = G::BN / 8;
    int lr = next_round(0), ik = 0, lnk = 0;
    unsigned goa[G::PA], gob[G::PB];
    const char* pa = nullptr;
    const char* pb = nullptr;
    unsigned long long ra_left = 0, rb_left = 0;
    unsigned sa = 0, sb = 0, fill = 0;
    auto setup = [&]() {
      const WsbItem it = g.items[(size_t)lr * nwg + wg];
      const WsbProb& P = g.p[it.prob];
      lnk = it.nk;
#pragma unroll
      for (int i = 0; i < G::PA; ++i) {
        const int id = (w * G::PA + i) * 64 + lane, row = id / CA, c = (id % CA) ^ swz_o<G::BM * 2>(row);
        goa[i] = (unsigned)row * (unsigned)P.lda * 2u + (c << 4);
      }
#pragma unroll
      for (int i = 0; i < G::PB; ++i) {
        const int id = (w * G::PB + i) * 64 + lane, row = id / CB, c = (id % CB) ^ swz_o<G::BN * 2>(row);
        gob[i] = (unsigned)row * (unsigned)P.ldb * 2u + (c << 4);
      }
      const int kb = it.k0 * 64;
      pa = reinterpret_cast<const char*>(P.A + (size_t)kb * P.lda + it.m0);
      pb = reinterpret_cast<const char*>(P.B + (size_t)kb * P.ldb + it.n0);
      ra_left = ((unsigned long long)(g.K - kb) * P.lda - it.m0) * 2;
      rb_left = ((unsigned long long)(g.K - kb) * P.ldb - it.n0) * 2;
      sa = 64u * (unsigned)P.lda * 2u;
      sb = 64u * (unsigned)P.ldb * 2u;
    };
    if (lr < g.rounds) setup();
    auto issue = [&]() -> bool {
      if (lr >= g.rounds) return false;
      char* buf = smem + fill;
      const __amdgpu_buffer_rsrc_t ra = __builtin_amdgcn_make_buffer_rsrc(const_cast<char*>(pa), 0, (unsigned)(ra_left < 0xfffffff0ull ? ra_left : 0xfffffff0ull), 0x00020000);
      const __amdgpu_buffer_rsrc_t rb = __builtin_amdgcn_make_buffer_rsrc(const_cast<char*>(pb), 0, (unsigned)(rb_left < 0xfffffff0ull ? rb_left : 0xfffffff0ull), 0x00020000);
#ifndef HERO_WSB_NOLOADS
#pragma unroll
      for (int i = 0; i < G::PA; ++i)
        __builtin_amdgcn_raw_ptr_buffer_load_lds(ra, HERO_LDS_PTR(buf + (w * G::PA + i) * 1024), 16, goa[i], 0, 0, HERO_WS_LOAD_AUX_A);
#pragma unroll
      for (int i = 0; i < G::PB; ++i)
        __builtin_amdgcn_raw_ptr_buffer_load_lds(rb, HERO_LDS_PTR(buf + G::A_BYTES + (w * G::PB + i) * 1024), 16, gob[i], 0, 0, HERO_WS_LOAD_AUX_B);
#else
      (void)ra; (void)rb; (void)buf;
#endif
      fill += G::STAGE;
      if (fill == NS * G::STAGE) fill = 0;
      if (++ik == lnk) {
        ik = 0;
        lr = next_round(lr + 1);
        if (lr < g.rounds) setup();
      } else {
        pa += sa; pb += sb;
        ra_left = ra_left > sa ? ra_left - sa : 0ull;
        rb_left = rb_left > sb ? rb_left - sb : 0ull;
      }
      return true;
    };
    issue();
    const bool second = issue();
    if (second) wait_vm<G::PW>(); else wait_vm<0>();
    __builtin_amdgcn_s_barrier();
    unsigned slot = 0;
    for (int r = next_round(0); r < g.rounds; r = next_round(r + 1)) {
      const WsbItem it = g.items[(size_t)r * nwg + wg];
      const bool want_cs = it.n0 == 0 && g.p[it.prob].colsum != nullptr;
      for (int t = 0; t < it.nk; ++t) {
        const bool more = issue();
        if (more) wait_vm<G::PW>(); else wait_vm<0>();
#ifndef HERO_WSB_NOBAR
        __builtin_amdgcn_s_barrier();
#endif
        if (t + 1 < it.nk) { slot += G::STAGE; if (slot == NS * G::STAGE) slot = 0; }
      }
#ifndef HERO_WSB_NOEPI
      epilogue_acc<G, false>(g.p[it.prob], it, g.flags, smem, slot, nullptr, wave, lane, want_cs);
#endif
      slot += G::STAGE; if (slot == NS * G::STAGE) slot = 0;
    }
    return;
  }

  const int wm = wave >> 1, wn = wave & 1;
  const int arow0 = wm * TM * 32, brow0 = wn * TN * 32;
  unsigned ao[TM], bo[TN];
  {
    const int p = lane & 15, gq = (lane >> 4) & 1, kg = lane >> 5;
    const int krow = kg * 8 + (p >> 2);
#pragma unroll
    for (int i = 0; i < TM; ++i) {
      const int col = arow0 + i * 32 + gq * 16 + 4 * (p & 3);
      ao[i] = krow * (G::BM * 2) + ((((col >> 3) ^ swz_o<G::BM * 2>(krow)) << 4) | ((col & 7) * 2));
    }
#pragma unroll
    for (int j = 0; j < TN; ++j) {
      const int col = brow0 + j * 32 + gq * 16 + 4 * (p & 3);
      bo[j] = G::A_BYTES + krow * (G::BN * 2) + ((((col >> 3) ^ swz_o<G::BN * 2>(krow)) << 4) | ((col & 7) * 2));
    }
  }
  typedef __attribute__((address_space(3))) bf16x4_t* lp_t;
  bf16x8_t a0[TM], b0[TN], a1[TM], b1[TN];
  auto ldf = [&](bf16x8_t (&a)[TM], bf16x8_t (&b)[TN], const char* st, int ks) {
#ifdef HERO_WSB_NOLDF
    return;
#endif
    auto ra = [&](int i) {
      const char* q = st + ao[i] + ks * 16 * (G::BM * 2);
      const bf16x4_t lo = __builtin_amdgcn_ds_read_tr16_b64_v4i16((lp_t)(q));
      const bf16x4_t hi = __builtin_amdgcn_ds_read_tr16_b64_v4i16((lp_t)(q + 4 * (G::BM * 2)));
      a[i] = bf16x8_t{lo[0], lo[1], lo[2], lo[3], hi[0], hi[1], hi[2], hi[3]};
    };
    ra(0);
#pragma unroll
    for (int j = 0; j < TN; ++j) {
      const char* q = st + bo[j] + ks * 16 * (G::BN * 2);
      const bf16x4_t lo = __builtin_amdgcn_ds_read_tr16_b64_v4i16((lp_t)(q));
      const bf16x4_t hi = __builtin_amdgcn_ds_read_tr16_b64_v4i16((lp_t)(q + 4 * (G::BN * 2)));
      b[j] = bf16x8_t{lo[0], lo[1], lo[2], lo[3], hi[0], hi[1], hi[2], hi[3]};
    }
#pragma unroll
    for (int i = 1; i < TM; ++i) ra(i);
  };
  f32x16_t acc[TM][TN];
  f32x16_t accb;
  unsigned selw[TM];
#pragma unroll
  for (int i = 0; i < TM; ++i) selw[i] = ((lane & 31) >> 3) == i ? 0x3f803f80u : 0u;
  auto mma = [&](const bf16x8_t (&a)[TM], const bf16x8_t (&b)[TN], auto cs) {
#ifdef HERO_WSB_NOMFMA
    asm volatile("" ::"v"(a[0]), "v"(b[0]), "v"(a[TM - 1]), "v"(b[TN - 1]));
    return;
#endif
#pragma unroll
    for (int i = 0; i < TM; ++i) {
#pragma unroll
      for (int j = 0; j < TN; ++j) acc[i][j] = __builtin_amdgcn_mfma_f32_32x32x16_bf16(b[j], a[i], acc[i][j], 0, 0, 0);
      if constexpr (decltype(cs)::value) {
        const u32x4_t w4 = {selw[i], selw[i], selw[i], selw[i]};
        accb = __builtin_amdgcn_mfma_f32_32x32x16_bf16(__builtin_bit_cast(bf16x8_t, w4), a[i], accb, 0, 0, 0);
      }
    }
  };
  unsigned curo = 0, last = 0;
  auto k_loop = [&](int nk, auto cs) {
    constexpr int NM = TM * TN + (decltype(cs)::value ? TM : 0);
    for (int t = 0; t < nk; ++t) {
      const char* cur = smem + curo;
      last = curo;
      curo += G::STAGE;
      if (curo == NS * G::STAGE) curo = 0;
      const char* nxt = smem + curo;
      ldf(a1, b1, cur, 1);
      mma(a0, b0, cs);
      WS_INTERLEAVE(NM, 2 * (TM + TN));
      __builtin_amdgcn_sched_barrier(0);
      ldf(a0, b0, cur, 2);
      mma(a1, b1, cs);
      WS_INTERLEAVE(NM, 2 * (TM + TN));
      __builtin_amdgcn_sched_barrier(0);
      ldf(a1, b1, cur, 3);
      mma(a0, b0, cs);
      WS_INTERLEAVE(NM, 2 * (TM + TN));
      __builtin_amdgcn_sched_barrier(0);
      wait_lds();
#ifndef HERO_WSB_NOBAR
      __builtin_amdgcn_s_barrier();
#endif
      __builtin_amdgcn_sched_barrier(0);
      ldf(a0, b0, nxt, 0);
      mma(a1, b1, cs);
      WS_INTERLEAVE(NM, 2 * (TM + TN));
      __builtin_amdgcn_sched_barrier(0);
    }
  };
  __builtin_amdgcn_s_setprio(2);
  __builtin_amdgcn_s_barrier();
  int r = next_round(0);
  if (r < g.rounds) ldf(a0, b0, smem, 0);
  while (r < g.rounds) {
    const WsbItem it = g.items[(size_t)r * nwg + wg];
    const int rn = next_round(r + 1);
    const bool cs_on = wn == 0 && it.n0 == 0 && g.p[it.prob].colsum != nullptr;
#pragma unroll
    for (int i = 0; i < TM; ++i)
#pragma unroll
      for (int j = 0; j < TN; ++j)
#pragma unroll
        for (int e = 0; e < 16; ++e) acc[i][j][e] = 0.f;
    last = curo;
    if (cs_on) {
#pragma unroll
      for (int e = 0; e < 16; ++e) accb[e] = 0.f;
      k_loop(it.nk, std::true_type{});
      float* sp = reinterpret_cast<float*>(smem + SPARE_OFF);
      if (lane < 32) {
#pragma unroll
        for (int i = 0; i < TM; ++i) sp[arow0 + 32 * i + lane] = accb[4 * i];
      }
    } else {
      k_loop(it.nk, std::false_type{});
    }
    __builtin_amdgcn_s_setprio(0);
#ifndef HERO_WSB_NOEPI
    epilogue_acc<G, true>(g.p[it.prob], it, g.flags, smem, last, acc, wave, lane);
#else
#pragma unroll
    for (int i = 0; i < TM; ++i)
#pragma unroll
      for (int j = 0; j < TN; ++j) asm volatile("" ::"v"(acc[i][j]));
#endif
    __builtin_amdgcn_s_setprio(2);
    if (rn < g.rounds) ldf(a0, b0, smem + curo, 0);
    r = rn;
  }
}

#define HERO_WS_INST(TM, TN)                                                                  \
  template __global__ void gemm_ws_kernel<TM, TN, false, 0>(WsArgs);                          \
  template __global__ void gemm_ws_kernel<TM, TN, false, EK_BIAS>(WsArgs);                    \
  template __global__ void gemm_ws_kernel<TM, TN, false, EK_BIAS | EK_RES | EK_DROP>(WsArgs); \
  template __global__ void gemm_ws_kernel<TM, TN, false, EK_BIAS | EK_GELU>(WsArgs);          \
  template __global__ void gemm_ws_kernel<TM, TN, false, EK_RES>(WsArgs);                     \
  template __global__ void gemm_ws_kernel<TM, TN, false, EK_GELU_BWD>(WsArgs);                \
  template __global__ void gemm_ws_kernel<TM, TN, true, 0>(WsArgs);
HERO_WS_INST(3, 3)
HERO_WS_INST(2, 3)

__global__ void ws_scale_f32_kernel(float* c, int M, int N, int ldc, float beta) {
  const size_t n4 = (size_t)N >> 2;
  for (size_t i = blockIdx.x * (size_t)blockDim.x + threadIdx.x; i < (size_t)M * n4; i += (size_t)gridDim.x * blockDim.x) {
    const size_t r = i / n4, c4 = (i - r * n4) * 4;
    float4* p = reinterpret_cast<float4*>(c + r * ldc + c4);
    if (beta == 0.f) {
      *p = make_float4(0.f, 0.f, 0.f, 0.f);
    } else {
      float4 v = *p;
      v.x *= beta; v.y *= beta; v.z *= beta; v.w *= beta;
      *p = v;
    }
  }
}

static int num_cus() {
  static int n = [] {
    int dev = 0, v = 256;
    if (hipGetDevice(&dev) == hipSuccess) (void)hipDeviceGetAttribute(&v, hipDeviceAttributeMultiprocessorCount, dev);
    return v > 0 ? v : 256;
  }();
  return n;
}

template <int TM, int TN, bool TR, int EK>
static int launch(WsArgs g, int slot, hipStream_t s) {
  typedef Geo<TM, TN> G;
  HERO_ENSURE_LDS((&gemm_ws_kernel<TM, TN, TR, EK>), G::LDS, "gemm_ws_kernel");
  const int grid = g.nwork < num_cus() ? g.nwork : num_cus();
  void* tok = gemm_prof_begin(slot, s);
  hipLaunchKernelGGL((gemm_ws_kernel<TM, TN, TR, EK>), dim3(grid), dim3(512), G::LDS, s, g);
  gemm_prof_end(tok, 2.0 * (double)g.M * (double)g.N * (double)g.K, s);
  return check_launch("hero_gemm(ws)");
}

template <int TM, int TN>
static int launch_kk(const WsArgs& g, hipStream_t s) {
  const HeroGemmEpilogue& e = g.epi;
  const bool b = e.bias != nullptr, r = e.residual != nullptr, d = e.dropout.threshold16 != 0;
  if (e.colsum != nullptr && e.act != HERO_ACT_GELU_BWD && e.act != HERO_ACT_MUL_AUX) return -1;
  if (e.act == HERO_ACT_NONE && b && !r && !d) return launch<TM, TN, false, EK_BIAS>(g, TM == 3 ? 8 : 10, s);
  if (e.act == HERO_ACT_NONE && b && r) return launch<TM, TN, false, EK_BIAS | EK_RES | EK_DROP>(g, TM == 3 ? 8 : 10, s);
  if ((e.act == HERO_ACT_GELU || e.act == HERO_ACT_GELU_DG) && b && !r && !d) return launch<TM, TN, false, EK_BIAS | EK_GELU>(g, TM == 3 ? 8 : 10, s);
  if (e.act == HERO_ACT_RELU && b && !r && !d && e.aux) return launch<TM, TN, false, EK_BIAS | EK_GELU>(g, TM == 3 ? 8 : 10, s);
  if constexpr (TM == 1) {
    if (e.act == HERO_ACT_RELU && b && r && !d && e.aux) return launch<TM, TN, false, EK_BIAS | EK_GELU | EK_RES>(g, 10, s);
  }
  if (e.act == HERO_ACT_NONE && !b && !r && !d) return launch<TM, TN, false, 0>(g, TM == 3 ? 8 : 10, s);
  if (e.act == HERO_ACT_NONE && !b && r && !d) return launch<TM, TN, false, EK_RES>(g, TM == 3 ? 8 : 10, s);
  if ((e.act == HERO_ACT_GELU_BWD || e.act == HERO_ACT_MUL_AUX) && !b && !r && !d) return launch<TM, TN, false, EK_GELU_BWD>(g, TM == 3 ? 8 : 10, s);
  return -1;
}

}

int gemm_ws_run(const void* A, const void* B, void* C, int M, int N, int K, int lda, int ldb, int ldc, int a_layout,
                int b_layout, const HeroGemmEpilogue& epi, int force_cfg, hipStream_t s) {
  using namespace ws;
  if (force_cfg == 8) return -1;
  if ((force_cfg < 9 || force_cfg > 14 || force_cfg == 11 || force_cfg == 12) && force_cfg != -1) return -1;
  typedef Geo<3, 3> G;
  const bool kk = a_layout == HERO_LAYOUT_K && b_layout == HERO_LAYOUT_K;
  const bool oo = a_layout == HERO_LAYOUT_O && b_layout == HERO_LAYOUT_O;
  if (!kk && !oo) return -1;
  if (K < 64 || N % 8 != 0 || M < 8) return -1;
  if ((force_cfg == 10 || force_cfg == 13 || force_cfg == 14) && !kk) return -1;
  WsArgs g;
  g.A = A; g.B = B; g.C = C;
  g.M = M; g.N = N; g.K = K; g.lda = lda; g.ldb = ldb; g.ldc = ldc;
  g.tiles_m = (M + G::BM - 1) / G::BM;
  g.tiles_n = (N + G::BN - 1) / G::BN;
  g.epi = epi;
  const int ntile = g.tiles_m * g.tiles_n;
  const int cus = num_cus();
  if (kk) {
    if (K % 64 != 0 || epi.out_f32 || epi.split_k > 1) return -1;
    if ((size_t)N * ldb * 2 >= 0x7fffffffull || (size_t)192 * lda * 2 >= 0x7fffffffull || (size_t)192 * ldc * 2 >= 0x7fffffffull) return -1;
    g.nsplit = 1;
    g.k_per_split = K;
    g.group = 8;
    typedef Geo<2, 3> G2;
    const int t23 = ((M + G2::BM - 1) / G2::BM) * g.tiles_n;
    const int r33 = (ntile + cus - 1) / cus, r23 = (t23 + cus - 1) / cus;
    const bool small = force_cfg == 10 || (force_cfg == -1 && r23 * 4 < r33 * 5 && t23 * 5 >= cus * 2);
    if (small) {
      g.tiles_m = (M + G2::BM - 1) / G2::BM;
      g.nwork = t23;
      return launch_kk<2, 3>(g, s);
    }
    if (force_cfg == 13 || force_cfg == 14 || (force_cfg == -1 && ntile * 2 < cus && K >= 512)) {
      typedef Geo<1, 2> G12;
      typedef Geo<1, 3> G13;
      const int rows64 = (M + 63) / 64;
      const int t12 = rows64 * ((N + G12::BN - 1) / G12::BN), t13 = rows64 * g.tiles_n;
      if (force_cfg == 14 || (force_cfg == -1 && t12 > cus && t13 <= cus)) {
        g.tiles_m = rows64; g.nwork = t13;
        return launch_kk<1, 3>(g, s);
      }
      if (force_cfg == 13 || (t12 * 8 >= cus && t12 <= cus)) {
        g.tiles_m = rows64; g.tiles_n = (N + G12::BN - 1) / G12::BN; g.nwork = t12;
        return launch_kk<1, 2>(g, s);
      }
    }
    if (force_cfg != 9 && ntile * 2 < cus) return -1;
    g.nwork = ntile;
    return launch_kk<3, 3>(g, s);
  }
  if (!epi.out_f32 || epi.act != HERO_ACT_NONE || epi.bias || epi.residual || epi.dropout.threshold16 != 0 || epi.colsum) return -1;
  if (M % 8 != 0) return -1;
  if ((size_t)K * lda * 2 >= 0xffffffffull || (size_t)K * ldb * 2 >= 0xffffffffull) return -1;
  const int ksteps = (K + 63) / 64;
  if (force_cfg != 9 && (ksteps < 32 || ntile < 64)) return -1;
  int split = cus / ntile;
  if (split > ksteps / 4) split = ksteps / 4;
  if (split < 1) split = 1;
  const int per = (ksteps + split - 1) / split;
  split = (ksteps + per - 1) / per;
  g.nsplit = split;
  g.k_per_split = per * 64;
  g.nwork = ntile * split;
  g.group = 8;
  if (epi.beta != 1.f) {
    hipLaunchKernelGGL(ws_scale_f32_kernel, dim3(1024), dim3(256), 0, s, static_cast<float*>(C), M, N, ldc, epi.beta);
    const int rc = check_launch("hero_gemm(ws scale)");
    if (rc) return rc;
  }
  return launch<3, 3, true, 0>(g, 9, s);
}

}

#ifdef HERO_WS_TRACE
extern "C" int hero_ws_trace_read(unsigned long long* out) {
  return hipMemcpyFromSymbol(out, HIP_SYMBOL(hero::ws::g_ws_trace), sizeof(unsigned long long) * 4 * 16 * 8) == hipSuccess ? 0 : -1;
}
#endif

extern "C" int hero_wgrad_group(const HeroWgradProblem* probs, int n, int K, int dtype, hero_stream_t stream) {
  using namespace hero;
  using namespace hero::ws;
  HERO_REQUIRE(probs && n >= 1 && n <= 4, "hero_wgrad_group: 1..4 problems");
  HERO_REQUIRE(dtype == HERO_BF16 || dtype == HERO_F32, "hero_wgrad_group: bad dtype %d", dtype);
  hipStream_t s = static_cast<hipStream_t>(stream);
  typedef Geo<3, 3> G;
  bool ok = dtype == HERO_BF16 && K >= 64 * 16 && gemm_forced_config() != 8;
  WsgArgs g;
  int tiles = 0;
  for (int i = 0; i < n && ok; ++i) {
    const HeroWgradProblem& q = probs[i];
    HERO_REQUIRE(q.dy && q.x && q.dw && q.M > 0 && q.N > 0, "hero_wgrad_group: bad problem %d", i);
    HERO_REQUIRE(q.dbias == nullptr, "hero_wgrad_group: dbias is a hero_wgrad_batch feature (problem %d)", i);
    ok = ok && q.M % 8 == 0 && q.N % 8 == 0 && q.ld_dy % 8 == 0 && q.ld_x % 8 == 0 && q.ld_dw % 4 == 0 &&
         (((uintptr_t)q.dy | (uintptr_t)q.x | (uintptr_t)q.dw) & 15) == 0 &&
         (size_t)K * q.ld_dy * 2 < 0xffffffffull && (size_t)K * q.ld_x * 2 < 0xffffffffull;
    WsgProb& P = g.p[i];
    P.A = static_cast<const bf16_t*>(q.dy); P.B = static_cast<const bf16_t*>(q.x); P.C = q.dw;
    P.M = q.M; P.N = q.N; P.lda = q.ld_dy; P.ldb = q.ld_x; P.ldc = q.ld_dw;
    P.tiles_n = (q.N + G::BN - 1) / G::BN;
    P.tile0 = tiles;
    tiles += ((q.M + G::BM - 1) / G::BM) * P.tiles_n;
  }
  const int ksteps = (K + 63) / 64;
  const int cus = num_cus();
  if (ok && (long long)tiles * ksteps >= 8LL * cus) {
    for (int i = n; i < 4; ++i) g.p[i] = g.p[0];
    g.nprob = n; g.K = K; g.ksteps = ksteps; g.total_tiles = tiles;
    HERO_ENSURE_LDS(&gemm_wsg_kernel, G::LDS, "gemm_wsg_kernel");
    double flops = 0.0;
    for (int i = 0; i < n; ++i) flops += 2.0 * probs[i].M * (double)probs[i].N * K;
    void* tok = gemm_prof_begin(9, s);
    hipLaunchKernelGGL(gemm_wsg_kernel, dim3(cus), dim3(512), G::LDS, s, g);
    gemm_prof_end(tok, flops, s);
    return check_launch("hero_wgrad_group");
  }
  for (int i = 0; i < n; ++i) {
    const HeroWgradProblem& q = probs[i];
    HeroGemmEpilogue e = {};
    e.out_f32 = 1; e.beta = 1.f; e.split_k = q.split_hint > 0 ? q.split_hint : 1; e.dropout.scale = 1.f;
    const int rc = hero_gemm(q.dy, q.x, q.dw, q.M, q.N, K, q.ld_dy, q.ld_x, q.ld_dw, HERO_LAYOUT_O, HERO_LAYOUT_O, dtype, &e, stream);
    if (rc) return rc;
  }
  return HERO_OK;
}

namespace hero {
namespace ws {
__device__ int g_wsb_flags[512];
constexpr int PLAN_MAGIC = 0x57534232;
constexpr int PLAN_HDR = 8;
}
}

extern "C" int hero_wgrad_batch_plan(const HeroWgradProblem* probs, int n, int K, int32_t* plan, int capacity_words) {
  using namespace hero;
  using namespace hero::ws;
  typedef Geo<3, 3> G;
  HERO_REQUIRE(probs && n >= 1 && n <= HERO_WGRAD_BATCH_MAX, "hero_wgrad_batch_plan: 1..%d problems", HERO_WGRAD_BATCH_MAX);
  HERO_REQUIRE(K >= 1, "hero_wgrad_batch_plan: K = %d", K);
  const int nwg = num_cus(), ksteps = (K + 63) / 64;
  if (nwg % 8 != 0 || ksteps < 8) return 0;
  struct T3 { int prob, mt, nt; };
  std::vector<T3> tiles;
  for (int i = 0; i < n; ++i) {
    HERO_REQUIRE(probs[i].M > 0 && probs[i].N > 0 && probs[i].M % 8 == 0 && probs[i].N % 8 == 0, "hero_wgrad_batch_plan: bad problem %d", i);
    const int tm = (probs[i].M + G::BM - 1) / G::BM, tn = (probs[i].N + G::BN - 1) / G::BN;
    const int per = nwg / 8;
    int pm = tm < 8 ? tm : 8;
    int pn = per / pm > 0 ? per / pm : 1;
    if (pn > tn) { pn = tn; pm = per / pn < tm ? per / pn : tm; if (pm < 1) pm = 1; }
    for (int bm = 0; bm < tm; bm += pm)
      for (int bn = 0; bn < tn; bn += pn)
        for (int mi = bm; mi < bm + pm && mi < tm; ++mi)
          for (int ni = bn; ni < bn + pn && ni < tn; ++ni) tiles.push_back({i, mi, ni});
  }
  const int T = (int)tiles.size();
  const int full = T / nwg, rem = T % nwg;
  struct Piece { int slot, round, tile, k0, nk, order, nslices; };
  std::vector<Piece> pieces;
  int tail_rounds = rem ? 1 : 0, S = 1;
  const int per_xcd_cap = nwg / 8, per_xcd = rem ? (rem + 7) / 8 : 0;
  if (rem) {
    HERO_REQUIRE(per_xcd <= 512 / 8, "hero_wgrad_batch_plan: flag capacity");
    for (int xcd = 0; xcd * per_xcd < rem; ++xcd) {
      const int t0 = xcd * per_xcd, p = (rem - t0 < per_xcd) ? rem - t0 : per_xcd, c = per_xcd_cap;
      int Sx = c / p;
      while (Sx > 1 && ksteps / Sx < 4) --Sx;
      if (Sx > 8) Sx = 8;
      auto cost_us = [&](int sl) { return (double)((ksteps + sl - 1) / sl) * 1.17 + (sl == 1 ? 8.0 : 9.0 + 16.0 * sl); };
      while (Sx > 1 && cost_us(Sx - 1) <= cost_us(Sx)) --Sx;
      const int L = c - Sx * p;
      const int E = 6;
      int q = (int)(((long long)p * ksteps + (long long)(p - L) * E + c - 1) / c);
      int r = ksteps - Sx * q;
      if (L == 0 || Sx != c / p || ksteps < 128 || r * 8 < ksteps) { r = 0; q = ksteps; }
      if (xcd == 0) S = Sx;
      std::vector<std::vector<Piece>> of_tile(p);
      int slot = Sx * p, fillq = 0, rnd = 0;
      for (int t = 0; t < p && r > 0; ++t) {
        int left = r;
        std::vector<Piece> mine;
        while (left > 0) {
          int room = q - fillq;
          if (slot >= c - 1) room = left;
          else if (room < 2 || (room < left && left - room < 2)) {
            if (room < 2) { ++slot; fillq = 0; rnd = 0; continue; }
            room = left;
          }
          const int take = left < room ? left : room;
          mine.push_back({slot < c ? slot : c - 1, rnd, t, 0, take, 0, 0});
          left -= take; fillq += take; ++rnd;
          if (fillq >= q && slot < c - 1) { ++slot; fillq = 0; rnd = 0; }
        }
        int k0 = 0, ord = 0;
        for (int i = (int)mine.size() - 1; i >= 0; --i) { mine[i].k0 = k0; mine[i].order = ord++; k0 += mine[i].nk; }
        of_tile[t] = mine;
      }
      for (int t = 0; t < p; ++t) {
        const int nrem = (int)of_tile[t].size();
        const int big0 = r;
        for (int sl = 0; sl < Sx; ++sl) {
          const int k0 = big0 + (int)((long long)(ksteps - big0) * sl / Sx), k1 = big0 + (int)((long long)(ksteps - big0) * (sl + 1) / Sx);
          of_tile[t].push_back({sl * p + t, 0, t, k0, k1 - k0, nrem + sl, 0});
        }
        for (Piece& pc : of_tile[t]) {
          pc.nslices = (int)of_tile[t].size();
          pc.slot += xcd * per_xcd_cap;
          pc.tile = t0 + t;
          if (pc.round + 1 > tail_rounds) tail_rounds = pc.round + 1;
          pieces.push_back(pc);
        }
      }
    }
  }
  const int rounds = full + tail_rounds;
  const int words = PLAN_HDR + rounds * nwg * 8;
  HERO_REQUIRE(plan && capacity_words >= words, "hero_wgrad_batch_plan: needs %d words, capacity %d", words, capacity_words);
  for (int i = PLAN_HDR; i < words; ++i) plan[i] = 0;
  auto item = [&](int r, int w) { return plan + PLAN_HDR + ((size_t)r * nwg + w) * 8; };
  for (int r = 0; r < full; ++r)
    for (int w = 0; w < nwg; ++w) {
      const T3& t = tiles[(size_t)r * nwg + w];
      int32_t* q = item(r, w);
      q[0] = t.prob; q[1] = t.mt * G::BM; q[2] = t.nt * G::BN; q[3] = 0; q[4] = ksteps; q[5] = 0; q[6] = 1; q[7] = 0;
    }
  for (const Piece& pc : pieces) {
    const T3& t = tiles[(size_t)full * nwg + pc.tile];
    int32_t* q = item(full + pc.round, pc.slot);
    HERO_REQUIRE(q[4] == 0, "hero_wgrad_batch_plan: internal error (slot used twice)");
    q[0] = t.prob; q[1] = t.mt * G::BM; q[2] = t.nt * G::BN; q[3] = pc.k0; q[4] = pc.nk; q[5] = pc.order; q[6] = pc.nslices;
    q[7] = (pc.slot / per_xcd_cap) * (512 / 8) + (pc.tile % per_xcd);
  }
  plan[0] = PLAN_MAGIC; plan[1] = nwg; plan[2] = rounds; plan[3] = rounds * nwg; plan[4] = n; plan[5] = K; plan[6] = T; plan[7] = S;
  return words;
}

extern "C" int hero_wgrad_batch(const HeroWgradProblem* probs, int n, int K, int dtype, const int32_t* plan_dev, int plan_words,
                                hero_stream_t stream) {
  using namespace hero;
  using namespace hero::ws;
  typedef Geo<3, 3> G;
  HERO_REQUIRE(probs && n >= 1 && n <= HERO_WGRAD_BATCH_MAX, "hero_wgrad_batch: 1..%d problems", HERO_WGRAD_BATCH_MAX);
  HERO_REQUIRE(dtype == HERO_BF16, "hero_wgrad_batch: bf16 only (dtype %d)", dtype);
  HERO_REQUIRE(plan_dev && plan_words > PLAN_HDR && (plan_words - PLAN_HDR) % (8 * num_cus()) == 0,
               "hero_wgrad_batch: the plan (%d words) was not made for this device (%d workgroups)", plan_words, num_cus());
  HERO_REQUIRE(((uintptr_t)plan_dev & 15) == 0, "hero_wgrad_batch: plan_dev must be 16-byte aligned");
  hipStream_t s = static_cast<hipStream_t>(stream);
  WsbArgs g;
  double flops = 0.0;
  for (int i = 0; i < n; ++i) {
    const HeroWgradProblem& q = probs[i];
    HERO_REQUIRE(q.dy && q.x && q.dw && q.M > 0 && q.N > 0 && q.M % 8 == 0 && q.N % 8 == 0 && q.ld_dy % 8 == 0 && q.ld_x % 8 == 0 &&
                     q.ld_dw % 4 == 0 && (((uintptr_t)q.dy | (uintptr_t)q.x | (uintptr_t)q.dw) & 15) == 0 &&
                     (size_t)64 * q.ld_dy * 2 < 0x7fffffffull && (size_t)64 * q.ld_x * 2 < 0x7fffffffull &&
                     (size_t)q.M * q.ld_dw * 4 < 0x7ffffff0ull,
                 "hero_wgrad_batch: problem %d is unaligned / too large", i);
    WsbProb& P = g.p[i];
    P.A = static_cast<const bf16_t*>(q.dy); P.B = static_cast<const bf16_t*>(q.x); P.C = q.dw;
    P.M = q.M; P.N = q.N; P.lda = q.ld_dy; P.ldb = q.ld_x; P.ldc = q.ld_dw; P.pad_ = 0;
    P.colsum = q.dbias;
    flops += 2.0 * q.M * (double)q.N * K;
  }
  for (int i = n; i < HERO_WGRAD_BATCH_MAX; ++i) g.p[i] = g.p[0];
  g.items = reinterpret_cast<const WsbItem*>(plan_dev + PLAN_HDR);
  g.rounds = (plan_words - PLAN_HDR) / (8 * num_cus());
  g.K = K; g.nprob = n; g.pad_ = 0;
  static int* flags_of[64] = {};
  int dev = 0;
  (void)hipGetDevice(&dev);
  HERO_REQUIRE(dev >= 0 && dev < 64, "hero_wgrad_batch: device %d", dev);
  if (!flags_of[dev]) HERO_REQUIRE(hipGetSymbolAddress(reinterpret_cast<void**>(&flags_of[dev]), HIP_SYMBOL(hero::ws::g_wsb_flags)) == hipSuccess,
                                   "hero_wgrad_batch: flag storage");
  g.flags = flags_of[dev];
  HERO_ENSURE_LDS(&gemm_wsb_kernel, G::LDS, "gemm_wsb_kernel");
  void* tok = gemm_prof_begin(9, s);
  hipLaunchKernelGGL(gemm_wsb_kernel, dim3(num_cus()), dim3(512), G::LDS, s, g);
  gemm_prof_end(tok, flops, s);
  return check_launch("hero_wgrad_batch");
}
```

hero_amd/csrc/gemm_ws_common.h:

```cpp
#pragma once
#include <vector>

#include "gemm_args.h"

namespace hero {
namespace ws {

typedef __attribute__((ext_vector_type(8))) short bf16x8_t;
typedef __attribute__((ext_vector_type(4))) short bf16x4_t;
typedef __attribute__((ext_vector_type(16))) float f32x16_t;
typedef __attribute__((ext_vector_type(4))) float f32x4_t;
typedef __attribute__((ext_vector_type(4))) unsigned u32x4_t;

constexpr int NS = 3;
constexpr int SPARE_OFF = 144 * 1024;

#ifndef HERO_WS_STORE_AUX
#define HERO_WS_STORE_AUX 2
#endif
#ifndef HERO_WS_STORE_AUX2
#define HERO_WS_STORE_AUX2 2
#endif
#ifndef HERO_WS_LOAD_AUX_A
#define HERO_WS_LOAD_AUX_A 0
#endif
#ifndef HERO_WS_LOAD_AUX_B
#define HERO_WS_LOAD_AUX_B 0
#endif
#ifndef HERO_WS_STORE_DW
#define HERO_WS_STORE_DW 0
#endif
#define HERO_LDS_PTR(p) ((__attribute__((address_space(3))) void*)(p))
template <int N> __device__ __forceinline__ void wait_vm() { asm volatile("s_waitcnt vmcnt(%0)" ::"n"(N) : "memory"); }
__device__ __forceinline__ void wait_lds() { asm volatile("s_waitcnt lgkmcnt(0)" ::: "memory"); }

template <int NM, int ND, int PER>
__device__ __forceinline__ void ws_interleave() {
#ifndef HERO_WS_BLOCKED
  if constexpr (NM > 0) {
    __builtin_amdgcn_sched_group_barrier(0x008, 1, 0);
    if constexpr (ND >= PER) __builtin_amdgcn_sched_group_barrier(0x100, PER, 0);
    else if constexpr (ND > 0) __builtin_amdgcn_sched_group_barrier(0x100, ND, 0);
    ws_interleave<NM - 1, (ND >= PER ? ND - PER : 0), PER>();
  }
#else
  __builtin_amdgcn_sched_group_barrier(0x100, ND, 0);
  __builtin_amdgcn_sched_group_barrier(0x008, NM, 0);
#endif
}
#define WS_INTERLEAVE(NM, ND) ws_interleave<(NM), (ND), ((ND) > (NM) ? 2 : 1)>()

#ifdef HERO_WS_TRACE
static __device__ unsigned long long g_ws_trace[4 * 16 * 8];
#define WS_T(item_no, ev, wave, lane)                                                                   \
  do {                                                                                                  \
    if (blockIdx.x == 0 && (lane) == 0 && (item_no) >= 0 && (item_no) < 4)                              \
      g_ws_trace[((item_no) * 16 + (ev)) * 8 + (wave)] = __builtin_readcyclecounter();                  \
  } while (0)
#else
#define WS_T(item_no, ev, wave, lane) do { } while (0)
#endif

struct WsArgs {
  const void* A;
  const void* B;
  void* C;
  int M, N, K, lda, ldb, ldc;
  int tiles_m, tiles_n, group, nsplit, k_per_split, nwork;
  HeroGemmEpilogue epi;
};

template <int TM_, int TN_> struct Geo {
  static constexpr int TM = TM_, TN = TN_;
  static constexpr int BM = 64 * TM, BN = 64 * TN;
  static constexpr int A_BYTES = BM * 128, B_BYTES = BN * 128, STAGE = A_BYTES + B_BYTES;
  static constexpr int PA = BM / 32, PB = BN / 32, PW = PA + PB;
  static constexpr int ROWB = BN * 4;
  static constexpr int RPP = (STAGE / ROWB >= 64 && BM % 64 == 0) ? 64 : 32;
  static constexpr int PASSES = BM / RPP;
  static constexpr int C8 = BN / 8, RPI = 512 / C8, ITERS = (RPP + RPI - 1) / RPI;
  static constexpr int NSG = SPARE_OFF / STAGE > 6 ? 6 : SPARE_OFF / STAGE;
  static constexpr int LDS = SPARE_OFF + 16384;
  static_assert(NSG >= 3 && NSG * STAGE <= SPARE_OFF && RPP * ROWB <= STAGE && RPI * BN * 4 <= 16384 && (NSG - 2) * PW < 64, "LDS budget");
  static_assert(TM_ < 2 || NSG == NS, "the large geometries keep the three-stage ring");
};

struct Item { int m0, n0, kbeg, nk; };

template <typename G>
__device__ __forceinline__ Item item_coord(const WsArgs& g, int item) {
  const int ntile = g.tiles_m * g.tiles_n;
  const int split = item / ntile;
  const int tile = item - split * ntile;
  const int per_group = g.group * g.tiles_n;
  const int group = tile / per_group;
  const int first_m = group * g.group;
  const int gsz = min(g.tiles_m - first_m, g.group);
  const int in_group = tile - group * per_group;
  Item it;
  it.m0 = (first_m + in_group % gsz) * G::BM;
  it.n0 = (in_group / gsz) * G::BN;
  it.kbeg = split * g.k_per_split;
  it.nk = (min(g.K, it.kbeg + g.k_per_split) - it.kbeg + 63) >> 6;
  return it;
}

__device__ __forceinline__ int swz_k(int row) { return (row ^ (row >> 3)) & 7; }
template <int RB> __device__ __forceinline__ int swz_o(int k) { return RB % 256 == 0 ? 4 * (k & 3) : 4 * ((k >> 1) & 1); }

template <typename G, bool TR>
struct Loader {
  const WsArgs& g;
  char* smem;
  int w, lane, nwg;
  int item, ik;
  Item ic;
  unsigned fill;
  unsigned goa[G::PA], gob[G::PB];
  const char* pa;
  const char* pb;
  unsigned ra_left, rb_left;

  __device__ __forceinline__ Loader(const WsArgs& g_, char* smem_, int wg, int nwg_, int w_, int lane_)
      : g(g_), smem(smem_), w(w_), lane(lane_), nwg(nwg_), item(wg), ik(0), fill(0) {
    if (item < g.nwork) setup();
  }
  __device__ __forceinline__ void setup() {
    ic = item_coord<G>(g, item);
    const bf16_t* A = static_cast<const bf16_t*>(g.A);
    const bf16_t* B = static_cast<const bf16_t*>(g.B);
    if (!TR) {
#pragma unroll
      for (int i = 0; i < G::PA; ++i) {
        const int r = (w * G::PA + i) * 8 + (lane >> 3);
        goa[i] = (unsigned)(min(ic.m0 + r, g.M - 1) - ic.m0) * (unsigned)g.lda * 2u + (((lane & 7) ^ swz_k(r)) << 4);
      }
#pragma unroll
      for (int i = 0; i < G::PB; ++i) {
        const int r = (w * G::PB + i) * 8 + (lane >> 3);
        gob[i] = (unsigned)(min(ic.n0 + r, g.N - 1) - ic.n0) * (unsigned)g.ldb * 2u + (((lane & 7) ^ swz_k(r)) << 4);
      }
      pa = reinterpret_cast<const char*>(A + (size_t)ic.m0 * g.lda + ic.kbeg);
      pb = reinterpret_cast<const char*>(B + (size_t)ic.n0 * g.ldb + ic.kbeg);
      ra_left = rb_left = 0x7fffffffu;
    } else {
      constexpr int CA = G::BM / 8, CB = G::BN / 8;
#pragma unroll
      for (int i = 0; i < G::PA; ++i) {
        const int id = (w * G::PA + i) * 64 + lane, row = id / CA, c = (id % CA) ^ swz_o<G::BM * 2>(row);
        goa[i] = (unsigned)row * (unsigned)g.lda * 2u + (c << 4);
      }
#pragma unroll
      for (int i = 0; i < G::PB; ++i) {
        const int id = (w * G::PB + i) * 64 + lane, row = id / CB, c = (id % CB) ^ swz_o<G::BN * 2>(row);
        gob[i] = (unsigned)row * (unsigned)g.ldb * 2u + (c << 4);
      }
      pa = reinterpret_cast<const char*>(A + (size_t)ic.kbeg * g.lda + ic.m0);
      pb = reinterpret_cast<const char*>(B + (size_t)ic.kbeg * g.ldb + ic.n0);
      ra_left = (unsigned)(((size_t)(g.K - ic.kbeg) * g.lda - ic.m0) * 2);
      rb_left = (unsigned)(((size_t)(g.K - ic.kbeg) * g.ldb - ic.n0) * 2);
    }
  }
  __device__ __forceinline__ void issue_always() {
    if (item >= g.nwork) { ra_left = rb_left = 0u; ic.nk = 0x7fffffff; }
    issue_body();
  }
  __device__ __forceinline__ bool issue() {
    if (item >= g.nwork) return false;
    issue_body();
    return true;
  }
  __device__ __forceinline__ void issue_body() {
    char* buf = smem + fill;
    const __amdgpu_buffer_rsrc_t ra = __builtin_amdgcn_make_buffer_rsrc(const_cast<char*>(pa), 0, ra_left, 0x00020000);
    const __amdgpu_buffer_rsrc_t rb = __builtin_amdgcn_make_buffer_rsrc(const_cast<char*>(pb), 0, rb_left, 0x00020000);
#pragma unroll
    for (int i = 0; i < G::PA; ++i)
      __builtin_amdgcn_raw_ptr_buffer_load_lds(ra, HERO_LDS_PTR(buf + (w * G::PA + i) * 1024), 16, goa[i], 0, 0, HERO_WS_LOAD_AUX_A);
#pragma unroll
    for (int i = 0; i < G::PB; ++i)
      __builtin_amdgcn_raw_ptr_buffer_load_lds(rb, HERO_LDS_PTR(buf + G::A_BYTES + (w * G::PB + i) * 1024), 16, gob[i], 0, 0, HERO_WS_LOAD_AUX_B);
    fill += G::STAGE;
    if (fill == G::NSG * G::STAGE) fill = 0;
    if (++ik == ic.nk) {
      item += nwg;
      ik = 0;
      if (item < g.nwork) setup();
    } else if (!TR) {
      pa += 128;
      pb += 128;
    } else {
      const unsigned sa = 64u * (unsigned)g.lda * 2u, sb = 64u * (unsigned)g.ldb * 2u;
      pa += sa; pb += sb;
      ra_left = ra_left > sa ? ra_left - sa : 0u;
      rb_left = rb_left > sb ? rb_left - sb : 0u;
    }
  }
};

template <typename G, int EK, bool COMPUTE>
__device__ __forceinline__ void epilogue_rows(const WsArgs& g, const Item& ic, char* smem, unsigned slot, f32x16_t (*acc)[G::TN], int wave,
                                              int lane, int trace_item = -1) {
  constexpr int TM = G::TM, TN = G::TN, BN = G::BN, RPP = G::RPP, C8 = G::C8, RPI = G::RPI, ITERS = G::ITERS;
  const HeroGemmEpilogue& e = g.epi;
  char* st = smem + slot;
  int tid = threadIdx.x;
  asm volatile("" : "+v"(tid));
  lane = tid & 63;
  wave = __builtin_amdgcn_readfirstlane(tid >> 6);
  const int c8 = tid % C8, r0 = tid / C8;
  const bool active = r0 < RPI;
  const int gn = ic.n0 + c8 * 8;
  const bool col_ok = active && gn < g.N;
  const int gnc = min(gn, g.N - 8);
  bf16_t* Cb = static_cast<bf16_t*>(g.C);
  const bf16_t* R = (EK & EK_RES) ? static_cast<const bf16_t*>(e.residual) : nullptr;
  bf16_t* X = static_cast<bf16_t*>(e.aux);
  const size_t torg = (size_t)ic.m0 * g.ldc + ic.n0;
  const __amdgpu_buffer_rsrc_t rsc = __builtin_amdgcn_make_buffer_rsrc(Cb + torg, 0, 0x7fffffff, 0x00020000);
  const __amdgpu_buffer_rsrc_t rsx = __builtin_amdgcn_make_buffer_rsrc((EK & EK_GELU) ? X + torg : Cb + torg, 0, 0x7fffffff, 0x00020000);
  DropCtx drop(e.dropout);
  const bool use_drop = (EK & EK_DROP) && drop.on();
  float bias[8] = {0.f, 0.f, 0.f, 0.f, 0.f, 0.f, 0.f, 0.f};
  if (EK & EK_BIAS) {
    const float4 b0 = *reinterpret_cast<const float4*>(e.bias + gnc);
    const float4 b1 = *reinterpret_cast<const float4*>(e.bias + gnc + 4);
    bias[0] = b0.x; bias[1] = b0.y; bias[2] = b0.z; bias[3] = b0.w;
    bias[4] = b1.x; bias[5] = b1.y; bias[6] = b1.z; bias[7] = b1.w;
  }
  const bool do_csum = (EK & EK_GELU_BWD) && e.colsum != nullptr;
  const bool save_dg = (EK & EK_GELU) && e.act == HERO_ACT_GELU_DG, mul_aux = (EK & EK_GELU_BWD) && e.act == HERO_ACT_MUL_AUX;
  const bool relu = (EK & EK_GELU) && e.act == HERO_ACT_RELU;
  float cs[8] = {0.f, 0.f, 0.f, 0.f, 0.f, 0.f, 0.f, 0.f};
  const int wm = wave >> 1, wn = wave & 1, l31 = lane & 31, half = lane >> 5;
  constexpr bool SPLIT = (RPP == 64 && G::PASSES == TM);
  auto tile_row = [](int p, int row) { return SPLIT ? (row >> 5) * (TM * 32) + p * 32 + (row & 31) : p * RPP + row; };

#pragma unroll
  for (int p = 0; p < G::PASSES; ++p) {
    uint4 pre[ITERS];
    unsigned off[ITERS];
    bool ok[ITERS];
#pragma unroll
    for (int it = 0; it < ITERS; ++it) {
      const int row = r0 + it * RPI;
      const int gm = ic.m0 + tile_row(p, row);
      ok[it] = col_ok && row < RPP && gm < g.M;
      off[it] = (unsigned)(min(gm, g.M - 1) - ic.m0) * (unsigned)g.ldc + (unsigned)(gnc - ic.n0);
      if (EK & EK_RES) pre[it] = *reinterpret_cast<const uint4*>(R + torg + off[it]);
      if (EK & EK_GELU_BWD) pre[it] = *reinterpret_cast<const uint4*>(X + torg + off[it]);
    }
    WS_T(trace_item, 2 + 4 * p, wave, lane);
    if constexpr (COMPUTE) {
#pragma unroll
      for (int b = 0; b < RPP / 32; ++b) {
        const int blk = SPLIT ? b * TM + p : p * (RPP / 32) + b;
        if (wm == blk / TM) {
          const int i = blk % TM;
#pragma unroll
          for (int j = 0; j < TN; ++j)
#pragma unroll
            for (int q = 0; q < 4; ++q) {
              const int chunk = (wn * TN * 32 + j * 32 + 8 * q + 4 * half) >> 2;
              const f32x4_t v = {acc[i][j][4 * q], acc[i][j][4 * q + 1], acc[i][j][4 * q + 2], acc[i][j][4 * q + 3]};
              *reinterpret_cast<f32x4_t*>(st + (32 * b + l31) * G::ROWB + ((chunk ^ (l31 & 7)) << 4)) = v;
            }
        }
      }
    }
    wait_lds();
    WS_T(trace_item, 3 + 4 * p, wave, lane);
    __builtin_amdgcn_s_barrier();
    WS_T(trace_item, 4 + 4 * p, wave, lane);
    uint4 outv[ITERS], auxv[(EK & EK_GELU) ? ITERS : 1];
#pragma unroll
    for (int it = 0; it < ITERS; ++it) {
      const int row = min(r0 + it * RPI, RPP - 1);
      {
        const int x = row & 7;
        const f32x4_t v0 = *reinterpret_cast<const f32x4_t*>(st + row * G::ROWB + (((2 * c8) ^ x) << 4));
        const f32x4_t v1 = *reinterpret_cast<const f32x4_t*>(st + row * G::ROWB + (((2 * c8 + 1) ^ x) << 4));
        float v[8] = {v0[0], v0[1], v0[2], v0[3], v1[0], v1[1], v1[2], v1[3]};
#pragma unroll
        for (int k = 0; k < 8; ++k) v[k] += bias[k];
        if (EK & EK_GELU) {
          uint4 u;
          if (save_dg) {
            float dg[8];
#pragma unroll
            for (int k = 0; k < 8; ++k) gelu_both<bf16_t>(v[k], v[k], dg[k]);
            u.x = f2bf_pk(dg[0], dg[1]); u.y = f2bf_pk(dg[2], dg[3]); u.z = f2bf_pk(dg[4], dg[5]); u.w = f2bf_pk(dg[6], dg[7]);
          } else if (relu) {
#pragma unroll
            for (int k = 0; k < 8; ++k) v[k] = fmaxf(v[k], 0.f);
            u.x = f2bf_pk(v[0], v[1]); u.y = f2bf_pk(v[2], v[3]); u.z = f2bf_pk(v[4], v[5]); u.w = f2bf_pk(v[6], v[7]);
          } else {
            u.x = f2bf_pk(v[0], v[1]); u.y = f2bf_pk(v[2], v[3]); u.z = f2bf_pk(v[4], v[5]); u.w = f2bf_pk(v[6], v[7]);
#pragma unroll
            for (int k = 0; k < 8; ++k) v[k] = gelu_fwd<bf16_t>(v[k]);
          }
          auxv[(EK & EK_GELU) ? it : 0] = u;
        }
        float pv[8];
        if (EK & (EK_RES | EK_GELU_BWD)) {
          const uint32_t w4[4] = {pre[it].x, pre[it].y, pre[it].z, pre[it].w};
#pragma unroll
          for (int k = 0; k < 4; ++k) {
            pv[2 * k] = __uint_as_float(w4[k] << 16);
            pv[2 * k + 1] = __uint_as_float(w4[k] & 0xffff0000u);
          }
        }
        if (EK & EK_GELU_BWD) {
          if (mul_aux) {
#pragma unroll
            for (int k = 0; k < 8; ++k) v[k] *= pv[k];
          } else {
#pragma unroll
            for (int k = 0; k < 8; ++k) v[k] *= gelu_grad<bf16_t>(pv[k]);
          }
        }
        if (use_drop) {
          const int gm = ic.m0 + tile_row(p, row);
          const uint64_t grp = ((uint64_t)gm * (uint64_t)g.N + (uint64_t)gn) >> 2;
          const float4 m0 = drop.mask4(grp), m1 = drop.mask4(grp + 1);
          v[0] *= m0.x; v[1] *= m0.y; v[2] *= m0.z; v[3] *= m0.w;
          v[4] *= m1.x; v[5] *= m1.y; v[6] *= m1.z; v[7] *= m1.w;
        }
        if (EK & EK_RES) {
#pragma unroll
          for (int k = 0; k < 8; ++k) v[k] += pv[k];
        }
        if (do_csum && ok[it]) {
#pragma unroll
          for (int k = 0; k < 8; ++k) cs[k] += v[k];
        }
        uint4 o;
        o.x = f2bf_pk(v[0], v[1]); o.y = f2bf_pk(v[2], v[3]); o.z = f2bf_pk(v[4], v[5]); o.w = f2bf_pk(v[6], v[7]);
        outv[it] = o;
      }
    }
#pragma unroll
    for (int it = 0; it < ITERS; ++it) {
      const unsigned vo = ok[it] ? (unsigned)(tile_row(p, r0 + it * RPI) * g.ldc + c8 * 8) * 2u : 0xffffffffu;
      if (EK & EK_GELU) {
        const uint4 u = auxv[(EK & EK_GELU) ? it : 0];
        __builtin_amdgcn_raw_buffer_store_b128(u32x4_t{u.x, u.y, u.z, u.w}, rsx, vo, 0, HERO_WS_STORE_AUX2);
      }
      __builtin_amdgcn_raw_buffer_store_b128(u32x4_t{outv[it].x, outv[it].y, outv[it].z, outv[it].w}, rsc, vo, 0, HERO_WS_STORE_AUX);
    }
    wait_lds();
    WS_T(trace_item, 5 + 4 * p, wave, lane);
    __builtin_amdgcn_s_barrier();
  }
  WS_T(trace_item, 14, wave, lane);
  if (EK & EK_GELU_BWD) {
    if (e.colsum != nullptr) {
      float* sp = reinterpret_cast<float*>(smem + SPARE_OFF);
      if (active) {
        *reinterpret_cast<f32x4_t*>(sp + r0 * BN + c8 * 8) = f32x4_t{cs[0], cs[1], cs[2], cs[3]};
        *reinterpret_cast<f32x4_t*>(sp + r0 * BN + c8 * 8 + 4) = f32x4_t{cs[4], cs[5], cs[6], cs[7]};
      }
      wait_lds();
      __builtin_amdgcn_s_barrier();
      if (tid < BN && ic.n0 + tid < g.N) {
        float t = 0.f;
#pragma unroll 4
        for (int k = 0; k < RPI; ++k) t += sp[k * BN + tid];
        if (e.colsum_partial) {
          float* pr = e.colsum + (size_t)(ic.m0 >> 6) * g.N + ic.n0 + tid;
          const int nb = min(G::BM >> 6, ((g.M + 63) >> 6) - (ic.m0 >> 6));
          pr[0] = t;
          for (int b = 1; b < nb; ++b) pr[(size_t)b * g.N] = 0.f;
        } else {
          atomicAdd(e.colsum + ic.n0 + tid, t);
        }
      }
    }
  }
}


}
}
```

include/hero_hip.h:

```cpp
#ifndef HERO_HIP_H_
#define HERO_HIP_H_

#include <stddef.h>
#include <stdint.h>

#ifdef __cplusplus
extern "C" {
#endif

typedef void* hero_stream_t;

enum { HERO_F32 = 0, HERO_BF16 = 1 };
enum { HERO_OK = 0, HERO_ERR_ARG = -1, HERO_ERR_LAUNCH = -2, HERO_ERR_UNSUPPORTED = -3 };

const char* hero_last_error(void);
#define HERO_ABI_VERSION 3
int hero_abi_version(void);
enum { HERO_STRUCT_DROPOUT = 0, HERO_STRUCT_GEMM_EPILOGUE, HERO_STRUCT_WGRAD_PROBLEM, HERO_STRUCT_LN_FWD, HERO_STRUCT_LN_BWD,
       HERO_STRUCT_COLSUM, HERO_STRUCT_ATTN, HERO_STRUCT_ADAMW, HERO_STRUCT_TENSOR_DESC, HERO_STRUCT_ADAMW_GROUP,
       HERO_STRUCT_ADAMW_MULTI, HERO_STRUCT_COPY_DESC, HERO_STRUCT_QUERY_POOL, HERO_STRUCT_ROW_NORM, HERO_STRUCT_SCORE_MAX,
       HERO_STRUCT_RANK_LOSS, HERO_STRUCT_ST_ED, HERO_STRUCT_CROSS_ENTROPY, HERO_STRUCT_DERIVE, HERO_STRUCT_COMM_BUCKET,
       HERO_STRUCT_COUNT_ };
int hero_abi_struct_count(void);
int hero_abi_struct_bytes(int which);

typedef struct HeroDropout {
  const uint64_t* seed_ptr;
  uint64_t site;
  uint32_t threshold16;
  float scale;
} HeroDropout;

enum { HERO_LAYOUT_K = 0,
       HERO_LAYOUT_O = 1   };
enum { HERO_ACT_NONE = 0,
       HERO_ACT_GELU = 1,
       HERO_ACT_RELU = 2,
       HERO_ACT_GELU_BWD = 3,
       HERO_ACT_RELU_BWD = 4,
       HERO_ACT_GELU_DG = 5,
       HERO_ACT_MUL_AUX = 6    };

typedef struct HeroGemmEpilogue {
  const float* bias;
  const void* residual;
  void* aux;
  int act;
  int out_f32;
  float beta;
  int split_k;
  HeroDropout dropout;
  float* colsum;
  int colsum_partial;
  int pad_;
  long long split_stride;
} HeroGemmEpilogue;

int hero_gemm(const void* A, const void* B, void* C, int M, int N, int K, int lda, int ldb, int ldc,
              int a_layout, int b_layout, int dtype, const HeroGemmEpilogue* epi, hero_stream_t stream);
int hero_gemm_splits(int K, int split_k, int dtype);
int hero_fold_slabs(const float* slabs, int n_slabs, size_t stride, void* out, size_t n, int out_dtype, hero_stream_t stream);

typedef struct HeroWgradProblem {
  const void* dy;
  const void* x;
  float* dw;
  int M, N, ld_dy, ld_x, ld_dw;
  int split_hint;
  float* dbias;
} HeroWgradProblem;
int hero_wgrad_group(const HeroWgradProblem* probs, int n, int K, int dtype, hero_stream_t stream);
#define HERO_WGRAD_BATCH_MAX 32
int hero_wgrad_batch_plan(const HeroWgradProblem* probs, int n, int K, int32_t* plan, int capacity_words);
int hero_wgrad_batch(const HeroWgradProblem* probs, int n, int K, int dtype, const int32_t* plan_dev, int plan_words,
                     hero_stream_t stream);
int hero_gemm_force_config(int cfg);
int hero_prof_enable(int on);
int hero_prof_read(int slot, double* total_ms, double* total_flops, long long* launches);

int hero_probe_mfma(void* scratch, size_t scratch_bytes, double* tflops, double* ghz, hero_stream_t stream);
int hero_probe_hbm(const void* src, void* dst, size_t bytes, double* copy_gbps, double* read_gbps, hero_stream_t stream);

typedef struct HeroLnFwd {
  const void* x;
  const float* tab[3];
  const int32_t* idx[3];
  const float* gamma;
  const float* beta;
  void* y;
  void* pre;
  float* mean;
  float* rstd;
  int rows, cols;
  float eps;
  int x_dtype, y_dtype;
  HeroDropout dropout;
} HeroLnFwd;
int hero_layernorm_fwd(const HeroLnFwd* a, hero_stream_t stream);

typedef struct HeroLnBwd {
  const void* x;
  const void* dy;
  const float* gamma;
  const float* mean;
  const float* rstd;
  void* dx;
  void* dx_dropped;
  float* dgamma;
  float* dbeta;
  float grad_beta;
  void* workspace;
  int rows, cols;
  int x_dtype, dtype;
  HeroDropout dropout_out;
  HeroDropout dropout_in;
  float* dbias_in;
  int defer_fold;
} HeroLnBwd;
size_t hero_layernorm_bwd_workspace_bytes(int rows, int cols);
int hero_layernorm_bwd_blocks(int rows);
int hero_layernorm_bwd(const HeroLnBwd* a, hero_stream_t stream);

size_t hero_colsum_workspace_bytes(int rows, int cols);
int hero_colsum(const void* x, float* out, int rows, int cols, int ld, int dtype, float beta,
                void* workspace, hero_stream_t stream);
#define HERO_COLSUM_MULTI_MAX 64
typedef struct HeroColsum {
  const void* src;
  float* dst;
  int rows, cols, ld, dtype;
  float beta;
  int row_cols;
  const int32_t* dst_rows;
} HeroColsum;
size_t hero_colsum_multi_workspace_bytes(const HeroColsum* p, int n);
int hero_colsum_multi(const HeroColsum* p, int n, void* workspace, hero_stream_t stream);

typedef struct HeroAttn {
  const void* qkv;
  const float* mask;
  void* ctx;
  float* probs;
  const void* dctx;
  void* dqkv;
  int S, L, H;
  float scale;
  int dtype;
  HeroDropout dropout;
  const int32_t* seq_off;
  float* stats;
} HeroAttn;
int hero_attention_fwd(const HeroAttn* a, hero_stream_t stream);
int hero_attention_bwd(const HeroAttn* a, hero_stream_t stream);
int hero_attention_max_len(int dtype, int backward);
int hero_attention_max_packed_len(int dtype);
int hero_attention_force_ppw(int ppw);
int hero_attention_stats_ok(int dtype, int L);

int hero_gather_rows(const void* a, const void* b, const int32_t* idx, void* out, int rows, int cols,
                     int dtype, hero_stream_t stream);
int hero_inverse_first(const int32_t* idx, int n, int32_t* inv, int na, int nb, hero_stream_t stream);
int hero_csr_gather_sum(const void* src, const int32_t* offsets, const int32_t* entries, void* out,
                        int rows, int cols, int dtype, hero_stream_t stream);
int hero_scatter_add_rows(const void* src, const int32_t* idx, void* dst_a, void* dst_b, int rows,
                          int cols, int src_dtype, int dst_dtype, int skip_idx, hero_stream_t stream);
size_t hero_segment_sort_workspace_bytes(int rows);
size_t hero_scatter_add_sorted_workspace_bytes(int rows, int cols);
int hero_segment_sort(const int32_t* idx, int rows, int n_dst, int skip_idx, int32_t* order, void* workspace,
                      hero_stream_t stream);
int hero_scatter_add_sorted(const void* src, const int32_t* idx, const int32_t* order, float* dst, int rows, int cols,
                            int src_dtype, int skip_idx, void* workspace, hero_stream_t stream);

int hero_cast(const void* src, void* dst, size_t n, int src_dtype, int dst_dtype, hero_stream_t stream);
int hero_transpose_cast(const float* src, void* dst, int rows, int cols, int ldd, int dst_dtype, hero_stream_t stream);
int hero_relu_bwd(const void* dy, const void* y, void* dx, size_t n, int dtype, hero_stream_t stream);
int hero_gelu_bwd(const void* dy, const void* u, void* dx, size_t n, int dtype, hero_stream_t stream);
int hero_add(const void* a, const void* b, void* y, size_t n, int dtype, hero_stream_t stream);

int hero_sumsq(const float* g, size_t n, float* sumsq, float* workspace, hero_stream_t stream);
typedef struct HeroAdamW {
  float* p;
  const float* g;
  float* m;
  float* v;
  size_t n;
  float lr, beta1, beta2, eps, weight_decay;
  int step;
  const float* grad_sumsq;
  float max_grad_norm;
  float grad_scale;
  void* shadow;
} HeroAdamW;
int hero_adamw(const HeroAdamW* a, hero_stream_t stream);

typedef struct HeroTensorDesc {
  float* p;
  const float* g;
  float* m;
  float* v;
  uint64_t n;
  int32_t group;
  int32_t step_lag;
} HeroTensorDesc;
typedef struct HeroAdamWGroup {
  float lr, beta1, beta2, eps, weight_decay;
} HeroAdamWGroup;
typedef struct HeroAdamWMulti {
  const HeroTensorDesc* descs;
  const int32_t* chunk_tensor;
  const int32_t* chunk_index;
  int n_chunks;
  HeroAdamWGroup groups[8];
  int step;
  const float* grad_sumsq;
  float max_grad_norm;
  float grad_scale;
  const int32_t* step_ptr;
  const float* lr_ptr;
  int32_t* tensor_steps;
  int n_tensors;
} HeroAdamWMulti;
int hero_adamw_multi(const HeroAdamWMulti* a, hero_stream_t stream);
int hero_adamw_multi_chunk(void);

typedef struct HeroCopyDesc {
  const float* src;
  void* dst;
  int32_t rows, cols, ldd;
  int32_t transpose;
  int32_t dst_dtype;
  int32_t pad_;
} HeroCopyDesc;
int hero_copy_multi(const HeroCopyDesc* descs, const int32_t* tile_desc, const int32_t* tile_index,
                    int n_tiles, hero_stream_t stream);

typedef struct HeroQueryPool {
  const void* q;
  const float* mask;
  const float* w;
  float* pooled;
  float* att;
  const float* dpooled;
  void* dq;
  float* dw;
  int B, L, D, dtype;
} HeroQueryPool;
int hero_query_pool_fwd(const HeroQueryPool* a, hero_stream_t stream);
int hero_query_pool_bwd(const HeroQueryPool* a, hero_stream_t stream);

int hero_qa_pool_fwd(const void* x, const float* mask, const float* w_qa, const float* w_se, float* qa_pooled, float* se_pooled,
                     float* att_qa, float* att_se, int Nv, int A, int L, int Lt, int D, int dtype, hero_stream_t stream);
int hero_qa_pool_bwd(const void* x, const float* mask, const float* w_qa, const float* w_se, const float* att_qa, const float* att_se,
                     const float* dqa, const float* dse, void* dx, float* dw_qa, float* dw_se,
                     int Nv, int A, int L, int Lt, int D, int dtype, hero_stream_t stream);

typedef struct HeroRowNorm {
  const void* x;
  float* y;
  float* rnorm;
  const float* dy;
  void* dx;
  int rows, cols, x_dtype;
  float eps;
} HeroRowNorm;
int hero_rownorm_fwd(const HeroRowNorm* a, hero_stream_t stream);
int hero_rownorm_bwd(const HeroRowNorm* a, hero_stream_t stream);

typedef struct HeroScoreMax {
  const float* s;
  const float* mask;
  float* out;
  int32_t* arg;
  const float* ds_ctx;
  const float* ds_q;
  const float* gc;
  const float* gq;
  const float* qn;
  const float* cn;
  float* dqn;
  float* dcn;
  int M, N, L, D, n0, n_own, ld_s;
  float gc_scale, gq_scale;
} HeroScoreMax;
int hero_sums_scaled(const float* src, int n_segs, int seg_len, const float* scales, float* out, hero_stream_t stream);
int hero_score_max_fwd(const HeroScoreMax* a, hero_stream_t stream);
int hero_score_max_bwd(const HeroScoreMax* a, hero_stream_t stream);

typedef struct HeroRankLoss {
  const float* s;
  float* loss_ctx_rows;
  float* loss_q_rows;
  float* ds_ctx;
  float* ds_q;
  int nq, nv;
  float margin;
  int lse;
  int hard;
  int pool;
  float hard_w, easy_w;
} HeroRankLoss;
int hero_rank_loss(const HeroRankLoss* a, hero_stream_t stream);

typedef struct HeroStEd {
  const float* q2;
  const void* ctx;
  const float* mask;
  const float* w_st;
  const float* w_ed;
  const int64_t* targets;
  float* loss_rows;
  float* p_st;
  float* p_ed;
  float* sim;
  const float* g;
  float* dq2;
  void* dctx;
  float* dw_st;
  float* dw_ed;
  int B, L, D, K, dtype;
  float g_scale;
  float* ws;
} HeroStEd;
size_t hero_st_ed_bwd_workspace_bytes(int B);
int hero_st_ed_fwd(const HeroStEd* a, hero_stream_t stream);
int hero_st_ed_bwd(const HeroStEd* a, hero_stream_t stream);

int hero_topk_rows(const float* scores, int M, int N, int ld, int k, float alpha, float* val, int* idx, hero_stream_t stream);
int hero_st_ed_probs(const float* sim, long long ld_sim, const float* mask, const int* sel, const float* w_st, const float* w_ed, int Nq,
                     int Nv, int K, int L, int taps, float* st_prob, float* ed_prob, hero_stream_t stream);
int hero_moment_topk(const float* st_prob, const float* ed_prob, const float* w, int Nq, int K, int L, int min_l, int max_l, int top_n,
                     float* score, int* flat, hero_stream_t stream);
int hero_moment_nms(const int* video, const int* st, const int* ed, int Nq, int N, double thd, int per_video_cap, int max_after, int* keep,
                    int* count, hero_stream_t stream);
int hero_first_hit(const int* video, const int* st, const int* ed, int Nq, int P, int ld, const int* gt_video, const float* gt_ts, float interval,
                   const float* thds, int T, int* first, hero_stream_t stream);

typedef struct HeroCrossEntropy {
  const void* logits;
  const int64_t* labels;
  float* loss;
  float* lse;
  const float* dloss;
  void* dlogits;
  int rows, cols, ld, dtype;
  float inv_temp;
  int64_t ignore_index;
} HeroCrossEntropy;
int hero_cross_entropy_fwd(const HeroCrossEntropy* a, hero_stream_t stream);
int hero_cross_entropy_bwd(const HeroCrossEntropy* a, hero_stream_t stream);

int hero_collate_subs(const int32_t* sub_nfrm, const int32_t* sub_ntok, int64_t* gather_index, int64_t* attn_mask, int T,
                      int max_vl, int out_size, hero_stream_t stream);
int hero_collate_gather_feats(const float* c_v_feats, float* f_v_feats, const int32_t* vid_sub_off, const int32_t* vid_nfrm,
                              const int32_t* sub_frm_off, const int32_t* sub_frm, int32_t* row_vid, int T, int max_vl, int B, int NF,
                              int D, hero_stream_t stream);
int hero_collate_clip_mask(const int32_t* vid_nfrm, int64_t* attn_mask, int B, int NF, hero_stream_t stream);
int hero_collate_frame_map(const int32_t* vid_sub_off, const int32_t* sub_frm_off, const int32_t* sub_frm, const int32_t* offsets,
                           int32_t* counts, int32_t* entries, int32_t* inverse, int B, int NF, int Lf, int fill,
                           hero_stream_t stream);

enum { HERO_DERIVE_MASK_ADD = 0, HERO_DERIVE_F32 = 1, HERO_DERIVE_I32 = 2, HERO_DERIVE_FLAT_GATHER = 3 };
#define HERO_DERIVE_MAX 16
typedef struct HeroDerive {
  const int64_t* src;
  void* dst;
  int64_t n;
  int mode;
  int p0, p1, p2;
} HeroDerive;
int hero_derive_multi(const HeroDerive* d, int n, hero_stream_t stream);

typedef struct HeroCommBucket {
  void* buf;
  size_t count;
  int dtype;
  int pad_;
} HeroCommBucket;
int hero_comm_available(void);
int hero_comm_unique_id(void* id128);
// ... 14 lines not shown
```

Before: 5325 videos/s.

## Add 64x96 and 64x64 warp-specialized GEMM tiles chosen by a cost model

Adds smaller output-tile geometries to the warp-specialized GEMM: a cut 64x96 variant (a 64x128 tile with a partial B half) and 64x64. When a GEMM has few large tiles relative to the CU count, a simple fill/epilogue time model picks among the existing geometry and the new ones. The goal is to reduce wave quantization and idle CUs on small-M or small-N GEMMs. The kernel body moves into a shared include so both kernel templates can use it, and the colsum epilogue reduction is reshaped for the 64-row case. The risks are model misprediction, which could pick a slower geometry, and more kernel instantiations to compile.

```diff
diff --git a/hero_amd/_lib.py b/hero_amd/_lib.py
--- a/hero_amd/_lib.py
+++ b/hero_amd/_lib.py
@@ -12,7 +12,7 @@
 ACT_NONE, ACT_GELU, ACT_RELU, ACT_GELU_BWD, ACT_RELU_BWD, ACT_GELU_DG, ACT_MUL_AUX = 0, 1, 2, 3, 4, 5, 6
 
 EXPORTS = [
-    "hero_last_error", "hero_abi_version", "hero_abi_struct_count", "hero_abi_struct_bytes", "hero_gemm", "hero_gemm_splits", "hero_fold_slabs", "hero_wgrad_group", "hero_wgrad_batch_plan", "hero_wgrad_batch", "hero_prof_enable", "hero_prof_read", "hero_probe_mfma", "hero_probe_hbm", "hero_gemm_force_config", "hero_layernorm_fwd",
+    "hero_last_error", "hero_abi_version", "hero_abi_struct_count", "hero_abi_struct_bytes", "hero_gemm", "hero_gemm_splits", "hero_fold_slabs", "hero_wgrad_group", "hero_wgrad_batch_plan", "hero_wgrad_batch", "hero_prof_enable", "hero_prof_read", "hero_probe_mfma", "hero_probe_hbm", "hero_gemm_force_config", "hero_gemm_ws_chosen_geometry", "hero_layernorm_fwd",
     "hero_layernorm_bwd_workspace_bytes", "hero_layernorm_bwd", "hero_colsum_workspace_bytes",
     "hero_colsum", "hero_colsum_multi", "hero_colsum_multi_workspace_bytes", "hero_layernorm_bwd_blocks", "hero_attention_fwd", "hero_attention_bwd", "hero_attention_max_len", "hero_attention_max_packed_len", "hero_attention_stats_ok", "hero_attention_force_ppw",
     "hero_gather_rows", "hero_inverse_first", "hero_csr_gather_sum", "hero_scatter_add_rows", "hero_segment_sort_workspace_bytes", "hero_scatter_add_sorted_workspace_bytes", "hero_segment_sort", "hero_scatter_add_sorted", "hero_cast", "hero_transpose_cast", "hero_copy_multi",
@@ -197,6 +197,7 @@
         L.hero_gemm.argtypes = [C.c_void_p, C.c_void_p, C.c_void_p] + [C.c_int] * 9 + [
             C.POINTER(GemmEpilogue), C.c_void_p]
         L.hero_gemm_splits.argtypes = [C.c_int, C.c_int, C.c_int]
+        L.hero_gemm_ws_chosen_geometry.argtypes = [C.c_int, C.c_int, C.c_int, C.POINTER(C.c_int), C.POINTER(C.c_int)]
         L.hero_fold_slabs.argtypes = [C.c_void_p, C.c_int, C.c_size_t, C.c_void_p, C.c_size_t, C.c_int, C.c_void_p]
         L.hero_wgrad_group.argtypes = [C.POINTER(WgradProblem), C.c_int, C.c_int, C.c_int, C.c_void_p]
         L.hero_wgrad_batch_plan.argtypes = [C.POINTER(WgradProblem), C.c_int, C.c_int, C.c_void_p, C.c_int]
diff --git a/hero_amd/build.py b/hero_amd/build.py
--- a/hero_amd/build.py
+++ b/hero_amd/build.py
@@ -30,7 +30,7 @@
 def build(force=False, verbose=False):
     os.makedirs(OBJ, exist_ok=True)
     hipcc = _hipcc()
-    headers = [os.path.join(CSRC, "common.h"), os.path.join(CSRC, "gemm_args.h"), os.path.join(CSRC, "gemm_ws_common.h"), os.path.join(CSRC, "attn_mfma.h"),
+    headers = [os.path.join(CSRC, "common.h"), os.path.join(CSRC, "gemm_args.h"), os.path.join(CSRC, "gemm_ws_common.h"), os.path.join(CSRC, "gemm_ws_kernel.inc"), os.path.join(CSRC, "attn_mfma.h"),
                os.path.join(os.path.dirname(HERE), "include", "hero_hip.h")]
     jobs = []
     objs = []
diff --git a/hero_amd/csrc/gemm.hip b/hero_amd/csrc/gemm.hip
--- a/hero_amd/csrc/gemm.hip
+++ b/hero_amd/csrc/gemm.hip
@@ -1083,7 +1083,7 @@
 }
 
 extern "C" int hero_gemm_force_config(int cfg) {
-  if (cfg >= 8 && cfg <= 14 && cfg != 11 && cfg != 12) {
+  if (cfg >= 8 && cfg <= 16 && cfg != 11 && cfg != 12) {
     g_force_cfg = cfg;
     g_use_glds = 1;
     g_group = 0;
diff --git a/hero_amd/csrc/gemm_ws.hip b/hero_amd/csrc/gemm_ws.hip
--- a/hero_amd/csrc/gemm_ws.hip
+++ b/hero_amd/csrc/gemm_ws.hip
@@ -9,191 +9,15 @@
 template <int TM, int TN, bool TR, int EK>
 __global__ __launch_bounds__(512) __attribute__((amdgpu_waves_per_eu(2, 2))) void gemm_ws_kernel(WsArgs g) {
   typedef Geo<TM, TN> G;
-  extern __shared__ __attribute__((aligned(16))) char smem[];
-  const int lane = threadIdx.x & 63;
-  const int wave = __builtin_amdgcn_readfirstlane(threadIdx.x >> 6);
-  const int nwg = gridDim.x;
-  int wg;
-  {
-    const int bid = blockIdx.x, q = nwg >> 3, r = nwg & 7, xcd = bid & 7, loc = bid >> 3;
-    wg = (xcd < r ? xcd * (q + 1) : r * (q + 1) + (xcd - r) * q) + loc;
-  }
-
-  if (wave >= 4) {
-    Loader<G, TR> ld(g, smem, wg, nwg, wave - 4, lane);
-    constexpr int AHEAD = (G::NSG - 2) * G::PW;
-    bool more = ld.issue();
-#pragma unroll
-    for (int k = 0; k < G::NSG - 2; ++k) more = ld.issue();
-    if (more) wait_vm<AHEAD>(); else wait_vm<0>();
-    __builtin_amdgcn_s_barrier();
-    unsigned slot = 0;
-    int item_no = 0;
-    for (int cit = wg; cit < g.nwork; cit += nwg, ++item_no) {
-      const Item ic = item_coord<G>(g, cit);
-      WS_T(item_no, 0, wave, lane);
-      for (int t = 0; t < ic.nk; ++t) {
-        if (ld.issue()) wait_vm<AHEAD>(); else wait_vm<0>();
-        __builtin_amdgcn_s_barrier();
-        if (t + 1 < ic.nk) { slot += G::STAGE; if (slot == G::NSG * G::STAGE) slot = 0; }
-      }
-      WS_T(item_no, 1, wave, lane);
-#ifndef HERO_WS_NOEPI
-      if constexpr (!TR) epilogue_rows<G, EK, false>(g, ic, smem, slot, nullptr, wave, lane, item_no);
-#endif
-      slot += G::STAGE; if (slot == G::NSG * G::STAGE) slot = 0;
-    }
-    return;
-  }
-
-  const int wm = wave >> 1, wn = wave & 1;
-  const int arow0 = wm * TM * 32, brow0 = wn * TN * 32;
-  unsigned ao[TM], bo[TN];
-  if (!TR) {
-    const int r = lane & 31, kg = lane >> 5;
-#pragma unroll
-    for (int i = 0; i < TM; ++i) { const int ra = arow0 + i * 32 + r; ao[i] = ra * 128 + ((kg ^ swz_k(ra)) << 4); }
-#pragma unroll
-    for (int j = 0; j < TN; ++j) { const int rb = brow0 + j * 32 + r; bo[j] = G::A_BYTES + rb * 128 + ((kg ^ swz_k(rb)) << 4); }
-  } else {
-    const int p = lane & 15, gq = (lane >> 4) & 1, kg = lane >> 5;
-    const int krow = kg * 8 + (p >> 2);
-#pragma unroll
-    for (int i = 0; i < TM; ++i) {
-      const int col = arow0 + i * 32 + gq * 16 + 4 * (p & 3);
-      ao[i] = krow * (G::BM * 2) + ((((col >> 3) ^ swz_o<G::BM * 2>(krow)) << 4) | ((col & 7) * 2));
-    }
-#pragma unroll
-    for (int j = 0; j < TN; ++j) {
-      const int col = brow0 + j * 32 + gq * 16 + 4 * (p & 3);
-      bo[j] = G::A_BYTES + krow * (G::BN * 2) + ((((col >> 3) ^ swz_o<G::BN * 2>(krow)) << 4) | ((col & 7) * 2));
-    }
-  }
-  bf16x8_t a0[TM], b0[TN], a1[TM], b1[TN];
-  auto ldf = [&](bf16x8_t (&a)[TM], bf16x8_t (&b)[TN], const char* st, int ks) {
-    typedef __attribute__((address_space(3))) bf16x4_t* lp_t;
-    auto ra = [&](int i) {
-      if (!TR) {
-        a[i] = *reinterpret_cast<const bf16x8_t*>(st + (ao[i] ^ (ks << 5)));
-      } else {
-        const char* q = st + ao[i] + ks * 16 * (G::BM * 2);
-        const bf16x4_t lo = __builtin_amdgcn_ds_read_tr16_b64_v4i16((lp_t)(q));
-        const bf16x4_t hi = __builtin_amdgcn_ds_read_tr16_b64_v4i16((lp_t)(q + 4 * (G::BM * 2)));
-        a[i] = bf16x8_t{lo[0], lo[1], lo[2], lo[3], hi[0], hi[1], hi[2], hi[3]};
-      }
-    };
-    auto rb = [&](int j) {
-      if (!TR) {
-        b[j] = *reinterpret_cast<const bf16x8_t*>(st + (bo[j] ^ (ks << 5)));
-      } else {
-        const char* q = st + bo[j] + ks * 16 * (G::BN * 2);
-        const bf16x4_t lo = __builtin_amdgcn_ds_read_tr16_b64_v4i16((lp_t)(q));
-        const bf16x4_t hi = __builtin_amdgcn_ds_read_tr16_b64_v4i16((lp_t)(q + 4 * (G::BN * 2)));
-        b[j] = bf16x8_t{lo[0], lo[1], lo[2], lo[3], hi[0], hi[1], hi[2], hi[3]};
-      }
-    };
-    if (!TR) {
-      ra(0);
-#pragma unroll
-      for (int j = 0; j < TN; ++j) rb(j);
-#pragma unroll
-      for (int i = 1; i < TM; ++i) ra(i);
-    } else {
-      ra(0);
-#pragma unroll
-      for (int j = 0; j < TN; ++j) rb(j);
-#pragma unroll
-      for (int i = 1; i < TM; ++i) ra(i);
-    }
-  };
-  f32x16_t acc[TM][TN];
-  auto mma = [&](const bf16x8_t (&a)[TM], const bf16x8_t (&b)[TN]) {
-#pragma unroll
-    for (int i = 0; i < TM; ++i)
-#pragma unroll
-      for (int j = 0; j < TN; ++j) {
-        if (!TR) acc[i][j] = __builtin_amdgcn_mfma_f32_32x32x16_bf16(b[j], a[i], acc[i][j], 0, 0, 0);
-        else acc[i][j] = __builtin_amdgcn_mfma_f32_32x32x16_bf16(a[i], b[j], acc[i][j], 0, 0, 0);
-      }
-  };
-
-  __builtin_amdgcn_s_setprio(2);
-  __builtin_amdgcn_s_barrier();
-  unsigned curo = 0;
-  if (wg < g.nwork) ldf(a0, b0, smem, 0);
-  int item_no = 0;
-  for (int cit = wg; cit < g.nwork; cit += nwg, ++item_no) {
-    const Item ic = item_coord<G>(g, cit);
-    WS_T(item_no, 0, wave, lane);
-#pragma unroll
-    for (int i = 0; i < TM; ++i)
-#pragma unroll
-      for (int j = 0; j < TN; ++j)
-#pragma unroll
-        for (int e = 0; e < 16; ++e) acc[i][j][e] = 0.f;
-    const bool more_items = cit + nwg < g.nwork;
-    unsigned last = curo;
-    for (int t = 0; t < ic.nk; ++t) {
-      const char* cur = smem + curo;
-      last = curo;
-      curo += G::STAGE;
-      if (curo == G::NSG * G::STAGE) curo = 0;
-      const char* nxt = smem + curo;
-      constexpr int NRD = TR ? 2 * (TM + TN) : TM + TN;
-      ldf(a1, b1, cur, 1);
-      mma(a0, b0);
-      WS_INTERLEAVE(TM * TN, NRD);
-      __builtin_amdgcn_sched_barrier(0);
-      ldf(a0, b0, cur, 2);
-      mma(a1, b1);
-      WS_INTERLEAVE(TM * TN, NRD);
-      __builtin_amdgcn_sched_barrier(0);
-      ldf(a1, b1, cur, 3);
-      mma(a0, b0);
-      WS_INTERLEAVE(TM * TN, NRD);
-      __builtin_amdgcn_sched_barrier(0);
-      wait_lds();
-      __builtin_amdgcn_s_barrier();
-      __builtin_amdgcn_sched_barrier(0);
-      ldf(a0, b0, nxt, 0);
-      mma(a1, b1);
-      WS_INTERLEAVE(TM * TN, NRD);
-      __builtin_amdgcn_sched_barrier(0);
-    }
-    if constexpr (!TR) {
-      __builtin_amdgcn_s_setprio(0);
-      WS_T(item_no, 1, wave, lane);
-#ifndef HERO_WS_NOEPI
-      epilogue_rows<G, EK, true>(g, ic, smem, last, acc, wave, lane, item_no);
-#else
-      {
-        float sum = 0.f;
-#pragma unroll
-        for (int i = 0; i < TM; ++i)
-#pragma unroll
-          for (int j = 0; j < TN; ++j)
-#pragma unroll
-            for (int e = 0; e < 16; ++e) sum += acc[i][j][e];
-        if (sum == 1.2345e-30f) static_cast<bf16_t*>(g.C)[lane] = (bf16_t)1;
-      }
-#endif
-      __builtin_amdgcn_s_setprio(2);
-      if (more_items) ldf(a0, b0, smem + curo, 0);
-    } else {
-      float* C = static_cast<float*>(g.C);
-#pragma unroll
-      for (int i = 0; i < TM; ++i)
-#pragma unroll
-        for (int j = 0; j < TN; ++j) {
-          const int gn = ic.n0 + brow0 + j * 32 + (lane & 31);
-#pragma unroll
-          for (int r = 0; r < 16; ++r) {
-            const int gm = ic.m0 + arow0 + i * 32 + (r & 3) + 8 * (r >> 2) + 4 * (lane >> 5);
-            if (gm < g.M && gn < g.N) atomicAdd(C + (size_t)gm * g.ldc + gn, acc[i][j][r]);
-          }
-        }
-    }
-  }
+#include "gemm_ws_kernel.inc"
+}
+
+template <int EK>
+__global__ __launch_bounds__(512) __attribute__((amdgpu_waves_per_eu(2, 2))) void gemm_ws_n96_kernel(WsArgs g) {
+  typedef Geo<1, 2, 1> G;
+  constexpr int TM = G::TM, TN = G::TN;
+  constexpr bool TR = false;
+#include "gemm_ws_kernel.inc"
 }
 
 struct WsgProb {
@@ -815,48 +639,109 @@
   return n;
 }
 
-template <int TM, int TN, bool TR, int EK>
+template <int TM, int TN, bool TR, int EK, int CUT = 0>
 static int launch(WsArgs g, int slot, hipStream_t s) {
-  typedef Geo<TM, TN> G;
-  HERO_ENSURE_LDS((&gemm_ws_kernel<TM, TN, TR, EK>), G::LDS, "gemm_ws_kernel");
+  typedef Geo<TM, TN, CUT> G;
+  void (*kern)(WsArgs);
+  if constexpr (CUT == 0) kern = gemm_ws_kernel<TM, TN, TR, EK>;
+  else kern = gemm_ws_n96_kernel<EK>;
+  static_assert(CUT == 0 || (TM == 1 && TN == 2 && !TR), "the only cut geometry is 64 x 96, K,K");
+  HERO_ENSURE_LDS(kern, G::LDS, "gemm_ws_kernel");
   const int grid = g.nwork < num_cus() ? g.nwork : num_cus();
   void* tok = gemm_prof_begin(slot, s);
-  hipLaunchKernelGGL((gemm_ws_kernel<TM, TN, TR, EK>), dim3(grid), dim3(512), G::LDS, s, g);
+  hipLaunchKernelGGL(kern, dim3(grid), dim3(512), G::LDS, s, g);
   gemm_prof_end(tok, 2.0 * (double)g.M * (double)g.N * (double)g.K, s);
   return check_launch("hero_gemm(ws)");
 }
 
-template <int TM, int TN>
+template <int TM, int TN, int CUT = 0>
 static int launch_kk(const WsArgs& g, hipStream_t s) {
   const HeroGemmEpilogue& e = g.epi;
   const bool b = e.bias != nullptr, r = e.residual != nullptr, d = e.dropout.threshold16 != 0;
   if (e.colsum != nullptr && e.act != HERO_ACT_GELU_BWD && e.act != HERO_ACT_MUL_AUX) return -1;
-  if (e.act == HERO_ACT_NONE && b && !r && !d) return launch<TM, TN, false, EK_BIAS>(g, TM == 3 ? 8 : 10, s);
-  if (e.act == HERO_ACT_NONE && b && r) return launch<TM, TN, false, EK_BIAS | EK_RES | EK_DROP>(g, TM == 3 ? 8 : 10, s);
-  if ((e.act == HERO_ACT_GELU || e.act == HERO_ACT_GELU_DG) && b && !r && !d) return launch<TM, TN, false, EK_BIAS | EK_GELU>(g, TM == 3 ? 8 : 10, s);
-  if (e.act == HERO_ACT_RELU && b && !r && !d && e.aux) return launch<TM, TN, false, EK_BIAS | EK_GELU>(g, TM == 3 ? 8 : 10, s);
+  if (e.act == HERO_ACT_NONE && b && !r && !d) return launch<TM, TN, false, EK_BIAS, CUT>(g, TM == 3 ? 8 : 10, s);
+  if (e.act == HERO_ACT_NONE && b && r) return launch<TM, TN, false, EK_BIAS | EK_RES | EK_DROP, CUT>(g, TM == 3 ? 8 : 10, s);
+  if ((e.act == HERO_ACT_GELU || e.act == HERO_ACT_GELU_DG) && b && !r && !d) return launch<TM, TN, false, EK_BIAS | EK_GELU, CUT>(g, TM == 3 ? 8 : 10, s);
+  if (e.act == HERO_ACT_RELU && b && !r && !d && e.aux) return launch<TM, TN, false, EK_BIAS | EK_GELU, CUT>(g, TM == 3 ? 8 : 10, s);
   if constexpr (TM == 1) {
-    if (e.act == HERO_ACT_RELU && b && r && !d && e.aux) return launch<TM, TN, false, EK_BIAS | EK_GELU | EK_RES>(g, 10, s);
-  }
-  if (e.act == HERO_ACT_NONE && !b && !r && !d) return launch<TM, TN, false, 0>(g, TM == 3 ? 8 : 10, s);
-  if (e.act == HERO_ACT_NONE && !b && r && !d) return launch<TM, TN, false, EK_RES>(g, TM == 3 ? 8 : 10, s);
-  if ((e.act == HERO_ACT_GELU_BWD || e.act == HERO_ACT_MUL_AUX) && !b && !r && !d) return launch<TM, TN, false, EK_GELU_BWD>(g, TM == 3 ? 8 : 10, s);
+    if (e.act == HERO_ACT_RELU && b && r && !d && e.aux) return launch<TM, TN, false, EK_BIAS | EK_GELU | EK_RES, CUT>(g, 10, s);
+  }
+  if (e.act == HERO_ACT_NONE && !b && !r && !d) return launch<TM, TN, false, 0, CUT>(g, TM == 3 ? 8 : 10, s);
+  if (e.act == HERO_ACT_NONE && !b && r && !d) return launch<TM, TN, false, EK_RES, CUT>(g, TM == 3 ? 8 : 10, s);
+  if ((e.act == HERO_ACT_GELU_BWD || e.act == HERO_ACT_MUL_AUX) && !b && !r && !d) return launch<TM, TN, false, EK_GELU_BWD, CUT>(g, TM == 3 ? 8 : 10, s);
   return -1;
 }
 
+}
+
+enum WsGeo { WS_NONE = 0, WS_192x192, WS_128x192, WS_64x128, WS_64x192, WS_64x96, WS_64x64 };
+
+static void ws_tile(int geo, int* bm, int* bn) {
+  static const int dims[7][2] = {{0, 0}, {192, 192}, {128, 192}, {64, 128}, {64, 192}, {64, 96}, {64, 64}};
+  *bm = dims[geo][0]; *bn = dims[geo][1];
+}
+static int ws_tiles(int geo, int M, int N) {
+  int bm, bn;
+  ws_tile(geo, &bm, &bn);
+  return ((M + bm - 1) / bm) * ((N + bn - 1) / bn);
+}
+
+static int ws_rounds_geo(int M, int N, int K, int force_cfg, int cus) {
+  const int ntile = ws_tiles(WS_192x192, M, N);
+  const int t23 = ws_tiles(WS_128x192, M, N);
+  const int r33 = (ntile + cus - 1) / cus, r23 = (t23 + cus - 1) / cus;
+  if (force_cfg == 10 || (force_cfg == -1 && r23 * 4 < r33 * 5 && t23 * 5 >= cus * 2)) return WS_128x192;
+  if (force_cfg == 13 || force_cfg == 14 || (force_cfg == -1 && ntile * 2 < cus && K >= 512)) {
+    const int t12 = ws_tiles(WS_64x128, M, N), t13 = ws_tiles(WS_64x192, M, N);
+    if (force_cfg == 14 || (force_cfg == -1 && t12 > cus && t13 <= cus)) return WS_64x192;
+    if (force_cfg == 13 || (t12 * 8 >= cus && t12 <= cus)) return WS_64x128;
+  }
+  if (force_cfg != 9 && ntile * 2 < cus) return WS_NONE;
+  return WS_192x192;
+}
+
+constexpr double WS_FILL_B_PER_US = 85.0e3;
+constexpr double WS_EPI_US_PER_PASS = 1.2;
+constexpr double WS_EPI_US_PER_ELEM = 0.04e-3;
+static double ws_model_us(int geo, int M, int N, int K, int cus) {
+  static const int passes[7] = {0, 3, 4, 1, 2, 2, 1};
+  int bm, bn;
+  ws_tile(geo, &bm, &bn);
+  const int tiles = ws_tiles(geo, M, N);
+  return (double)((tiles + cus - 1) / cus) *
+         ((double)(K / 64) * (bm + bn) * 128.0 / WS_FILL_B_PER_US + WS_EPI_US_PER_PASS * passes[geo] + WS_EPI_US_PER_ELEM * bm * bn);
+}
+
+static int ws_choose_geo(int M, int N, int K, int force_cfg, int cus) {
+  if (force_cfg == 15) return WS_64x96;
+  if (force_cfg == 16) return WS_64x64;
+  int geo = ws_rounds_geo(M, N, K, force_cfg, cus);
+  if (force_cfg != -1 || geo == WS_NONE || geo == WS_192x192 || ws_tiles(WS_192x192, M, N) > cus) return geo;
+  double best = ws_model_us(geo, M, N, K, cus);
+  for (int cand : {(int)WS_64x96, (int)WS_64x64}) {
+    const double t = ws_model_us(cand, M, N, K, cus);
+    if (t < best) { best = t; geo = cand; }
+  }
+  return geo;
+}
+
+static bool ws_kk_ok(int M, int N, int K, int lda, int ldb, int ldc, const HeroGemmEpilogue& epi) {
+  if (K < 64 || N % 8 != 0 || M < 8) return false;
+  if (K % 64 != 0 || epi.out_f32 || epi.split_k > 1) return false;
+  return !((size_t)N * ldb * 2 >= 0x7fffffffull || (size_t)192 * lda * 2 >= 0x7fffffffull || (size_t)192 * ldc * 2 >= 0x7fffffffull);
 }
 
 int gemm_ws_run(const void* A, const void* B, void* C, int M, int N, int K, int lda, int ldb, int ldc, int a_layout,
                 int b_layout, const HeroGemmEpilogue& epi, int force_cfg, hipStream_t s) {
   using namespace ws;
   if (force_cfg == 8) return -1;
-  if ((force_cfg < 9 || force_cfg > 14 || force_cfg == 11 || force_cfg == 12) && force_cfg != -1) return -1;
+  if ((force_cfg < 9 || force_cfg > 16 || force_cfg == 11 || force_cfg == 12) && force_cfg != -1) return -1;
   typedef Geo<3, 3> G;
   const bool kk = a_layout == HERO_LAYOUT_K && b_layout == HERO_LAYOUT_K;
   const bool oo = a_layout == HERO_LAYOUT_O && b_layout == HERO_LAYOUT_O;
   if (!kk && !oo) return -1;
   if (K < 64 || N % 8 != 0 || M < 8) return -1;
-  if ((force_cfg == 10 || force_cfg == 13 || force_cfg == 14) && !kk) return -1;
+  if ((force_cfg == 10 || force_cfg >= 13) && !kk) return -1;
   WsArgs g;
   g.A = A; g.B = B; g.C = C;
   g.M = M; g.N = N; g.K = K; g.lda = lda; g.ldb = ldb; g.ldc = ldc;
@@ -866,37 +751,25 @@
   const int ntile = g.tiles_m * g.tiles_n;
   const int cus = num_cus();
   if (kk) {
-    if (K % 64 != 0 || epi.out_f32 || epi.split_k > 1) return -1;
-    if ((size_t)N * ldb * 2 >= 0x7fffffffull || (size_t)192 * lda * 2 >= 0x7fffffffull || (size_t)192 * ldc * 2 >= 0x7fffffffull) return -1;
+    if (!ws_kk_ok(M, N, K, lda, ldb, ldc, epi)) return -1;
     g.nsplit = 1;
     g.k_per_split = K;
     g.group = 8;
-    typedef Geo<2, 3> G2;
-    const int t23 = ((M + G2::BM - 1) / G2::BM) * g.tiles_n;
-    const int r33 = (ntile + cus - 1) / cus, r23 = (t23 + cus - 1) / cus;
-    const bool small = force_cfg == 10 || (force_cfg == -1 && r23 * 4 < r33 * 5 && t23 * 5 >= cus * 2);
-    if (small) {
-      g.tiles_m = (M + G2::BM - 1) / G2::BM;
-      g.nwork = t23;
-      return launch_kk<2, 3>(g, s);
-    }
-    if (force_cfg == 13 || force_cfg == 14 || (force_cfg == -1 && ntile * 2 < cus && K >= 512)) {
-      typedef Geo<1, 2> G12;
-      typedef Geo<1, 3> G13;
-      const int rows64 = (M + 63) / 64;
-      const int t12 = rows64 * ((N + G12::BN - 1) / G12::BN), t13 = rows64 * g.tiles_n;
-      if (force_cfg == 14 || (force_cfg == -1 && t12 > cus && t13 <= cus)) {
-        g.tiles_m = rows64; g.nwork = t13;
-        return launch_kk<1, 3>(g, s);
-      }
-      if (force_cfg == 13 || (t12 * 8 >= cus && t12 <= cus)) {
-        g.tiles_m = rows64; g.tiles_n = (N + G12::BN - 1) / G12::BN; g.nwork = t12;
-        return launch_kk<1, 2>(g, s);
-      }
-    }
-    if (force_cfg != 9 && ntile * 2 < cus) return -1;
-    g.nwork = ntile;
-    return launch_kk<3, 3>(g, s);
+    const int geo = ws_choose_geo(M, N, K, force_cfg, cus);
+    if (geo == WS_NONE) return -1;
+    int bm, bn;
+    ws_tile(geo, &bm, &bn);
+    g.tiles_m = (M + bm - 1) / bm;
+    g.tiles_n = (N + bn - 1) / bn;
+    g.nwork = g.tiles_m * g.tiles_n;
+    switch (geo) {
+      case WS_128x192: return launch_kk<2, 3>(g, s);
+      case WS_64x128: return launch_kk<1, 2>(g, s);
+      case WS_64x192: return launch_kk<1, 3>(g, s);
+      case WS_64x96: return launch_kk<1, 2, 1>(g, s);
+      case WS_64x64: return launch_kk<1, 1>(g, s);
+      default: return launch_kk<3, 3>(g, s);
+    }
   }
   if (!epi.out_f32 || epi.act != HERO_ACT_NONE || epi.bias || epi.residual || epi.dropout.threshold16 != 0 || epi.colsum) return -1;
   if (M % 8 != 0) return -1;
@@ -920,6 +793,18 @@
   return launch<3, 3, true, 0>(g, 9, s);
 }
 
+}
+
+extern "C" int hero_gemm_ws_chosen_geometry(int M, int N, int K, int* bm, int* bn) {
+  using namespace hero;
+  using namespace hero::ws;
+  HERO_REQUIRE(bm && bn && M > 0 && N > 0 && K > 0, "hero_gemm_ws_chosen_geometry: bad argument");
+  HeroGemmEpilogue e = {};
+  const int f = gemm_forced_config();
+  const bool ws_forced = f == -1 || f == 9 || f == 10 || (f >= 13 && f <= 16);
+  const int geo = ws_forced && ws_kk_ok(M, N, K, K, K, N, e) ? ws_choose_geo(M, N, K, f, num_cus()) : WS_NONE;
+  ws_tile(geo, bm, bn);
+  return HERO_OK;
 }
 
 #ifdef HERO_WS_TRACE
diff --git a/hero_amd/csrc/gemm_ws_common.h b/hero_amd/csrc/gemm_ws_common.h
--- a/hero_amd/csrc/gemm_ws_common.h
+++ b/hero_amd/csrc/gemm_ws_common.h
@@ -70,9 +70,9 @@
   HeroGemmEpilogue epi;
 };
 
-template <int TM_, int TN_> struct Geo {
+template <int TM_, int TN_, int CUT_ = 0> struct Geo {
   static constexpr int TM = TM_, TN = TN_;
-  static constexpr int BM = 64 * TM, BN = 64 * TN;
+  static constexpr int BM = 64 * TM, BN = 64 * TN - 32 * CUT_;
   static constexpr int A_BYTES = BM * 128, B_BYTES = BN * 128, STAGE = A_BYTES + B_BYTES;
   static constexpr int PA = BM / 32, PB = BN / 32, PW = PA + PB;
   static constexpr int ROWB = BN * 4;
@@ -83,6 +83,7 @@
   static constexpr int LDS = SPARE_OFF + 16384;
   static_assert(NSG >= 3 && NSG * STAGE <= SPARE_OFF && RPP * ROWB <= STAGE && RPI * BN * 4 <= 16384 && (NSG - 2) * PW < 64, "LDS budget");
   static_assert(TM_ < 2 || NSG == NS, "the large geometries keep the three-stage ring");
+  static_assert(CUT_ == 0 || (CUT_ == 1 && TN_ >= 2), "a cut tile drops the last fragment of the right wave column");
 };
 
 struct Item { int m0, n0, kbeg, nk; };
@@ -258,13 +259,15 @@
         if (wm == blk / TM) {
           const int i = blk % TM;
 #pragma unroll
-          for (int j = 0; j < TN; ++j)
+          for (int j = 0; j < TN; ++j) {
+            if (BN < 64 * TN && wn * TN * 32 + j * 32 >= BN) continue;
 #pragma unroll
             for (int q = 0; q < 4; ++q) {
               const int chunk = (wn * TN * 32 + j * 32 + 8 * q + 4 * half) >> 2;
               const f32x4_t v = {acc[i][j][4 * q], acc[i][j][4 * q + 1], acc[i][j][4 * q + 2], acc[i][j][4 * q + 3]};
               *reinterpret_cast<f32x4_t*>(st + (32 * b + l31) * G::ROWB + ((chunk ^ (l31 & 7)) << 4)) = v;
             }
+          }
         }
       }
     }
@@ -364,8 +367,13 @@
       __builtin_amdgcn_s_barrier();
       if (tid < BN && ic.n0 + tid < g.N) {
         float t = 0.f;
+        if constexpr (G::BM == 64 && RPI == 64) {
 #pragma unroll 4
-        for (int k = 0; k < RPI; ++k) t += sp[k * BN + tid];
+          for (int k = 0; k < 32; ++k) t += sp[k * BN + tid] + sp[(k + 32) * BN + tid];
+        } else {
+#pragma unroll 4
+          for (int k = 0; k < RPI; ++k) t += sp[k * BN + tid];
+        }
         if (e.colsum_partial) {
           float* pr = e.colsum + (size_t)(ic.m0 >> 6) * g.N + ic.n0 + tid;
           const int nb = min(G::BM >> 6, ((g.M + 63) >> 6) - (ic.m0 >> 6));
diff --git a/hero_amd/csrc/gemm_ws_kernel.inc b/hero_amd/csrc/gemm_ws_kernel.inc
--- /dev/null
+++ b/hero_amd/csrc/gemm_ws_kernel.inc
@@ -0,0 +1,188 @@
+  extern __shared__ __attribute__((aligned(16))) char smem[];
+  const int lane = threadIdx.x & 63;
+  const int wave = __builtin_amdgcn_readfirstlane(threadIdx.x >> 6);
+  const int nwg = gridDim.x;
+  int wg;
+  {
+    const int bid = blockIdx.x, q = nwg >> 3, r = nwg & 7, xcd = bid & 7, loc = bid >> 3;
+    wg = (xcd < r ? xcd * (q + 1) : r * (q + 1) + (xcd - r) * q) + loc;
+  }
+
+  if (wave >= 4) {
+    Loader<G, TR> ld(g, smem, wg, nwg, wave - 4, lane);
+    constexpr int AHEAD = (G::NSG - 2) * G::PW;
+    bool more = ld.issue();
+#pragma unroll
+    for (int k = 0; k < G::NSG - 2; ++k) more = ld.issue();
+    if (more) wait_vm<AHEAD>(); else wait_vm<0>();
+    __builtin_amdgcn_s_barrier();
+    unsigned slot = 0;
+    int item_no = 0;
+    for (int cit = wg; cit < g.nwork; cit += nwg, ++item_no) {
+      const Item ic = item_coord<G>(g, cit);
+      WS_T(item_no, 0, wave, lane);
+      for (int t = 0; t < ic.nk; ++t) {
+        if (ld.issue()) wait_vm<AHEAD>(); else wait_vm<0>();
+        __builtin_amdgcn_s_barrier();
+        if (t + 1 < ic.nk) { slot += G::STAGE; if (slot == G::NSG * G::STAGE) slot = 0; }
+      }
+      WS_T(item_no, 1, wave, lane);
+#ifndef HERO_WS_NOEPI
+      if constexpr (!TR) epilogue_rows<G, EK, false>(g, ic, smem, slot, nullptr, wave, lane, item_no);
+#endif
+      slot += G::STAGE; if (slot == G::NSG * G::STAGE) slot = 0;
+    }
+    return;
+  }
+
+  const int wm = wave >> 1, wn = wave & 1;
+  const int arow0 = wm * TM * 32, brow0 = wn * TN * 32;
+  unsigned ao[TM], bo[TN];
+  if (!TR) {
+    const int r = lane & 31, kg = lane >> 5;
+#pragma unroll
+    for (int i = 0; i < TM; ++i) { const int ra = arow0 + i * 32 + r; ao[i] = ra * 128 + ((kg ^ swz_k(ra)) << 4); }
+#pragma unroll
+    for (int j = 0; j < TN; ++j) {
+      const int rb = (G::BN < 64 * TN && brow0 + j * 32 >= G::BN ? brow0 : brow0 + j * 32) + r;
+      bo[j] = G::A_BYTES + rb * 128 + ((kg ^ swz_k(rb)) << 4);
+    }
+  } else {
+    const int p = lane & 15, gq = (lane >> 4) & 1, kg = lane >> 5;
+    const int krow = kg * 8 + (p >> 2);
+#pragma unroll
+    for (int i = 0; i < TM; ++i) {
+      const int col = arow0 + i * 32 + gq * 16 + 4 * (p & 3);
+      ao[i] = krow * (G::BM * 2) + ((((col >> 3) ^ swz_o<G::BM * 2>(krow)) << 4) | ((col & 7) * 2));
+    }
+#pragma unroll
+    for (int j = 0; j < TN; ++j) {
+      const int col = brow0 + j * 32 + gq * 16 + 4 * (p & 3);
+      bo[j] = G::A_BYTES + krow * (G::BN * 2) + ((((col >> 3) ^ swz_o<G::BN * 2>(krow)) << 4) | ((col & 7) * 2));
+    }
+  }
+  bf16x8_t a0[TM], b0[TN], a1[TM], b1[TN];
+  auto ldf = [&](bf16x8_t (&a)[TM], bf16x8_t (&b)[TN], const char* st, int ks) {
+    typedef __attribute__((address_space(3))) bf16x4_t* lp_t;
+    auto ra = [&](int i) {
+      if (!TR) {
+        a[i] = *reinterpret_cast<const bf16x8_t*>(st + (ao[i] ^ (ks << 5)));
+      } else {
+        const char* q = st + ao[i] + ks * 16 * (G::BM * 2);
+        const bf16x4_t lo = __builtin_amdgcn_ds_read_tr16_b64_v4i16((lp_t)(q));
+        const bf16x4_t hi = __builtin_amdgcn_ds_read_tr16_b64_v4i16((lp_t)(q + 4 * (G::BM * 2)));
+        a[i] = bf16x8_t{lo[0], lo[1], lo[2], lo[3], hi[0], hi[1], hi[2], hi[3]};
+      }
+    };
+    auto rb = [&](int j) {
+      if (!TR) {
+        b[j] = *reinterpret_cast<const bf16x8_t*>(st + (bo[j] ^ (ks << 5)));
+      } else {
+        const char* q = st + bo[j] + ks * 16 * (G::BN * 2);
+        const bf16x4_t lo = __builtin_amdgcn_ds_read_tr16_b64_v4i16((lp_t)(q));
+        const bf16x4_t hi = __builtin_amdgcn_ds_read_tr16_b64_v4i16((lp_t)(q + 4 * (G::BN * 2)));
+        b[j] = bf16x8_t{lo[0], lo[1], lo[2], lo[3], hi[0], hi[1], hi[2], hi[3]};
+      }
+    };
+    if (!TR) {
+      ra(0);
+#pragma unroll
+      for (int j = 0; j < TN; ++j) rb(j);
+#pragma unroll
+      for (int i = 1; i < TM; ++i) ra(i);
+    } else {
+      ra(0);
+#pragma unroll
+      for (int j = 0; j < TN; ++j) rb(j);
+#pragma unroll
+      for (int i = 1; i < TM; ++i) ra(i);
+    }
+  };
+  f32x16_t acc[TM][TN];
+  auto mma = [&](const bf16x8_t (&a)[TM], const bf16x8_t (&b)[TN]) {
+#pragma unroll
+    for (int i = 0; i < TM; ++i)
+#pragma unroll
+      for (int j = 0; j < TN; ++j) {
+        if (!TR) acc[i][j] = __builtin_amdgcn_mfma_f32_32x32x16_bf16(b[j], a[i], acc[i][j], 0, 0, 0);
+        else acc[i][j] = __builtin_amdgcn_mfma_f32_32x32x16_bf16(a[i], b[j], acc[i][j], 0, 0, 0);
+      }
+  };
+
+  __builtin_amdgcn_s_setprio(2);
+  __builtin_amdgcn_s_barrier();
+  unsigned curo = 0;
+  if (wg < g.nwork) ldf(a0, b0, smem, 0);
+  int item_no = 0;
+  for (int cit = wg; cit < g.nwork; cit += nwg, ++item_no) {
+    const Item ic = item_coord<G>(g, cit);
+    WS_T(item_no, 0, wave, lane);
+#pragma unroll
+    for (int i = 0; i < TM; ++i)
+#pragma unroll
+      for (int j = 0; j < TN; ++j)
+#pragma unroll
+        for (int e = 0; e < 16; ++e) acc[i][j][e] = 0.f;
+    const bool more_items = cit + nwg < g.nwork;
+    unsigned last = curo;
+    for (int t = 0; t < ic.nk; ++t) {
+      const char* cur = smem + curo;
+      last = curo;
+      curo += G::STAGE;
+      if (curo == G::NSG * G::STAGE) curo = 0;
+      const char* nxt = smem + curo;
+      constexpr int NRD = TR ? 2 * (TM + TN) : TM + TN;
+      ldf(a1, b1, cur, 1);
+      mma(a0, b0);
+      WS_INTERLEAVE(TM * TN, NRD);
+      __builtin_amdgcn_sched_barrier(0);
+      ldf(a0, b0, cur, 2);
+      mma(a1, b1);
+      WS_INTERLEAVE(TM * TN, NRD);
+      __builtin_amdgcn_sched_barrier(0);
+      ldf(a1, b1, cur, 3);
+      mma(a0, b0);
+      WS_INTERLEAVE(TM * TN, NRD);
+      __builtin_amdgcn_sched_barrier(0);
+      wait_lds();
+      __builtin_amdgcn_s_barrier();
+      __builtin_amdgcn_sched_barrier(0);
+      ldf(a0, b0, nxt, 0);
+      mma(a1, b1);
+      WS_INTERLEAVE(TM * TN, NRD);
+      __builtin_amdgcn_sched_barrier(0);
+    }
+    if constexpr (!TR) {
+      __builtin_amdgcn_s_setprio(0);
+      WS_T(item_no, 1, wave, lane);
+#ifndef HERO_WS_NOEPI
+      epilogue_rows<G, EK, true>(g, ic, smem, last, acc, wave, lane, item_no);
+#else
+      {
+        float sum = 0.f;
+#pragma unroll
+        for (int i = 0; i < TM; ++i)
+#pragma unroll
+          for (int j = 0; j < TN; ++j)
+#pragma unroll
+            for (int e = 0; e < 16; ++e) sum += acc[i][j][e];
+        if (sum == 1.2345e-30f) static_cast<bf16_t*>(g.C)[lane] = (bf16_t)1;
+      }
+#endif
+      __builtin_amdgcn_s_setprio(2);
+      if (more_items) ldf(a0, b0, smem + curo, 0);
+    } else {
+      float* C = static_cast<float*>(g.C);
+#pragma unroll
+      for (int i = 0; i < TM; ++i)
+#pragma unroll
+        for (int j = 0; j < TN; ++j) {
+          const int gn = ic.n0 + brow0 + j * 32 + (lane & 31);
+#pragma unroll
+          for (int r = 0; r < 16; ++r) {
+            const int gm = ic.m0 + arow0 + i * 32 + (r & 3) + 8 * (r >> 2) + 4 * (lane >> 5);
+            if (gm < g.M && gn < g.N) atomicAdd(C + (size_t)gm * g.ldc + gn, acc[i][j][r]);
+          }
+        }
+    }
+  }
diff --git a/include/hero_hip.h b/include/hero_hip.h
--- a/include/hero_hip.h
+++ b/include/hero_hip.h
@@ -75,6 +75,7 @@
 int hero_wgrad_batch(const HeroWgradProblem* probs, int n, int K, int dtype, const int32_t* plan_dev, int plan_words,
                      hero_stream_t stream);
 int hero_gemm_force_config(int cfg);
+int hero_gemm_ws_chosen_geometry(int M, int N, int K, int* bm, int* bn);
 int hero_prof_enable(int on);
 int hero_prof_read(int slot, double* total_ms, double* total_flops, long long* launches);
 
```

Result: no change. 5365 videos/s, median of 6 (+0.8%).
